# laiviet/ed-gated-gcn

Measured on AMD Instinct MI355X. Metric: gated_gcn_forward_edges_per_sec, higher is better.
Workload: dtype f32 (fp16 MFMA + block-scaled fp8 correction MFMA, fp32 accumulate)

## Files before the change

### ed-gated-gcn_amd/_capi.py

```python
import ctypes
import os

_HERE = os.path.dirname(os.path.abspath(__file__))
_LIB = None

c_i32, c_i64, c_vp, c_sz = ctypes.c_int, ctypes.c_int64, ctypes.c_void_p, ctypes.c_size_t

PROTOTYPES = {
    "ggcn_abi_version": (c_i32, []),
    "ggcn_has_f16mx6": (c_i32, []),
    "ggcn_last_error": (ctypes.c_char_p, []),
    "ggcn_csr_workspace_bytes": (c_sz, [c_i64]),
    "ggcn_csr_from_dense": (c_i32, [c_vp, c_i32, c_i32, c_i32, c_i64, c_i64, c_i64, c_vp, c_vp, c_vp,
                                    c_i64, c_vp, c_vp, c_vp, c_vp]),
    "ggcn_rowmask_from_dense": (c_i32, [c_vp, c_i32, c_i32, c_i32, c_i64, c_i64, c_i64, c_vp, c_vp, c_vp]),
    "ggcn_csr_transpose": (c_i32, [c_vp, c_vp, c_vp, c_i32, c_i32, c_vp, c_vp, c_vp, c_vp, c_vp]),
    "ggcn_csr_rowmask": (c_i32, [c_vp, c_vp, c_i32, c_i32, c_vp, c_vp]),
    "ggcn_graph_edge_lists_bytes": (c_sz, [c_i32]),
    "ggcn_graph_edge_lists": (c_i32, [c_vp, c_i32, c_i32, c_vp, c_vp]),
    "ggcn_graph_operands_bytes": (c_sz, [c_i32]),
    "ggcn_graph_operands": (c_i32, [c_vp, c_i32, c_i32, c_vp, c_vp]),
    "ggcn_graph_operands2_bytes": (c_sz, [c_i32]),
    "ggcn_graph_operands2": (c_i32, [c_vp, c_i32, c_i32, c_i32, c_vp, c_vp]),
    "ggcn_graph_operands_weighted": (c_i32, [c_vp, c_vp, c_vp, c_i32, c_i32, c_i32, c_vp, c_vp, c_vp]),
    "ggcn_layer_fused_weighted": (c_i32, [c_vp, c_i64, c_vp, c_vp, c_vp, c_vp, c_i32, c_i32, c_i32, c_i32, c_vp, c_vp, c_vp,
                                          c_vp, c_i64, c_vp, c_vp, c_vp, c_vp, c_vp, c_i32, c_vp]),
    "ggcn_graph_operands_weighted_wide_bytes": (c_sz, [c_i32, c_i32]),
    "ggcn_graph_operands_weighted_wide": (c_i32, [c_vp, c_vp, c_vp, c_i32, c_i32, c_vp, c_vp, c_vp]),
    "ggcn_layer_fused_weighted_wide": (c_i32, [c_vp, c_i64, c_vp, c_vp, c_vp, c_i32, c_i32, c_i32, c_i32, c_vp, c_vp, c_vp,
                                               c_vp, c_i64, c_vp, c_vp, c_i32, c_vp]),
    "ggcn_layer_fused_weighted_drop": (c_i32, [c_vp, c_i64, c_vp, c_vp, c_vp, c_vp, c_i32, c_i32, c_i32, c_i32, c_vp, c_vp, c_vp,
                                               c_vp, c_i64, c_vp, c_vp, c_i32, ctypes.c_float, ctypes.c_uint64, c_i32, c_i32, c_i32, c_vp]),
    "ggcn_layer_fused_weighted_wide_drop": (c_i32, [c_vp, c_i64, c_vp, c_vp, c_vp, c_i32, c_i32, c_i32, c_i32, c_vp, c_vp, c_vp,
                                                    c_vp, c_i64, c_vp, c_vp, c_i32, ctypes.c_float, ctypes.c_uint64, c_i32, c_i32, c_i32, c_vp]),
    "ggcn_layer_fused": (c_i32, [c_vp, c_i64, c_vp, c_vp, c_vp, c_vp, c_i32, c_i32, c_i32, c_i32, c_vp, c_vp, c_vp,
                                 c_vp, c_i64, c_vp, c_vp, c_vp, c_vp, c_vp, c_i32, c_vp]),
    "ggcn_layer_fused_prebias": (c_i32, [c_vp, c_i64, c_vp, c_vp, c_vp, c_vp, c_i32, c_i32, c_i32, c_i32, c_vp, c_vp, c_vp,
                                         c_vp, c_i64, c_vp, c_vp, c_i32, c_vp]),
    "ggcn_block_fused": (c_i32, [c_vp, c_i64, c_vp, c_vp, c_vp, c_vp, c_vp, c_vp, c_vp, c_i32, c_i32, c_i32, c_i32,
                                 c_vp, c_vp, c_vp, c_i64, c_vp, c_i64, c_vp, c_vp, c_vp, c_vp, c_i32, c_vp]),
    "ggcn_graph_operands2_weighted": (c_i32, [c_vp, c_vp, c_vp, c_i32, c_i32, c_i32, c_vp, c_vp, c_vp]),
    "ggcn_block_fused_weighted": (c_i32, [c_vp, c_i64, c_vp, c_vp, c_vp, c_vp, c_vp, c_vp, c_vp, c_vp, c_i32, c_i32, c_i32, c_i32,
                                          c_vp, c_vp, c_vp, c_i64, c_vp, c_i64, c_vp, c_vp, c_vp, c_vp, c_i32, c_vp]),
    "ggcn_overlap_reduce": (c_i32, [c_vp, c_i32, c_i32, c_vp, c_vp]),
    "ggcn_transpose": (c_i32, [c_vp, c_i32, c_i32, c_i64, c_vp, c_vp]),
    "ggcn_gate_mlp": (c_i32, [c_vp, c_i64, c_i32, c_i32, c_vp, c_vp, c_vp, c_vp, c_vp, c_vp, c_vp, c_vp, c_vp, c_vp, c_vp]),
    "ggcn_scores_head": (c_i32, [c_vp, c_i64, c_vp, c_i64, c_vp, c_i64, c_vp, c_i64, c_vp, c_vp, c_i64, c_i32, c_i32,
                                 c_i32, c_i32, c_vp, c_i64, c_vp, c_vp]),
    "ggcn_absmax": (c_i32, [c_vp, c_i32, c_i64, c_i64, c_i32, c_vp, c_vp]),
    "ggcn_range_flag": (c_i32, [c_vp, c_i32, c_vp]),
    "ggcn_debug_poison_lds": (c_i32, [ctypes.c_uint32, c_vp]),
    "ggcn_lab_block_fused8": (c_i32, [c_vp, c_i64, c_vp, c_vp, c_vp, c_vp, c_vp, c_vp, c_vp, c_i32, c_i32, c_i32, c_i32, c_vp, c_vp,
                                      c_vp, c_i64, c_vp, c_vp, c_vp, c_vp, c_vp, c_vp]),
    "ggcn_debug_mfma_calibrate": (c_i32, [c_i32, c_i32, c_vp, c_vp, c_vp]),
    "ggcn_debug_block_fused_stamped": (c_i32, [c_vp, c_i64, c_vp, c_vp, c_vp, c_vp, c_vp, c_vp, c_vp, c_i32, c_i32, c_i32, c_i32,
                                               c_vp, c_vp, c_vp, c_i64, c_vp, c_i64, c_vp, c_vp, c_vp, c_vp, c_i32, c_vp, c_vp]),
    "ggcn_subword_pool": (c_i32, [c_vp, c_i64, c_i64, c_i64, c_vp, c_i64, c_i64, c_vp, c_i64, c_i64,
                                  c_i32, c_i32, c_i32, c_i32, c_vp]),
    "ggcn_subword_pool_bf16": (c_i32, [c_vp, c_i64, c_i64, c_i64, c_vp, c_i64, c_i64, c_vp, c_i64, c_i64,
                                       c_i32, c_i32, c_i32, c_i32, c_vp]),
    "ggcn_linear_bf16": (c_i32, [c_vp, c_i64, c_vp, c_vp, c_i64, c_i64, c_i32, c_i32, c_vp]),
    "ggcn_linear_out_bf16": (c_i32, [c_vp, c_i64, c_vp, c_vp, c_i64, c_i64, c_i32, c_i32, c_vp]),
    "ggcn_layer_fused_bf16": (c_i32, [c_vp, c_i64, c_vp, c_vp, c_vp, c_i32, c_i32, c_i32, c_i32, c_vp, c_vp, c_vp,
                                      c_vp, c_i64, c_vp, c_vp, c_vp, c_vp, c_vp, c_vp]),
    "ggcn_layer_fused_bf16_drop": (c_i32, [c_vp, c_i64, c_vp, c_vp, c_vp, c_i32, c_i32, c_i32, c_i32, c_vp, c_vp, c_vp,
                                           c_vp, c_i64, c_vp, c_vp, c_vp, c_vp, c_vp,
                                           ctypes.c_float, ctypes.c_uint64, c_i32, c_i32, c_i32, c_vp]),
    "ggcn_layer_fused_bf16_wide": (c_i32, [c_vp, c_i64, c_vp, c_vp, c_vp, c_vp, c_i32, c_i32, c_i32, c_i32, c_vp, c_vp, c_vp,
                                           c_vp, c_i64, c_vp, c_vp, c_vp, c_vp, c_vp,
                                           ctypes.c_float, ctypes.c_uint64, c_i32, c_i32, c_i32, c_vp]),
    "ggcn_block_fused_bf16": (c_i32, [c_vp, c_i64, c_vp, c_vp, c_vp, c_vp, c_vp, c_vp, c_vp, c_i32, c_i32, c_i32, c_i32,
                                      c_vp, c_vp, c_vp, c_i64, c_vp, c_i64, c_vp, c_vp, c_vp, c_vp, c_vp]),
    "ggcn_aggregate_bf16": (c_i32, [c_vp, c_i64, c_vp, c_vp, c_vp, c_i32, c_i32, c_i32, c_vp, c_i64, c_vp]),
    "ggcn_dweight_bf16_workspace_bytes": (c_sz, [c_i64, c_i32, c_i32]),
    "ggcn_dweight_bf16": (c_i32, [c_vp, c_i64, c_vp, c_i64, c_i64, c_i32, c_i32, c_vp, c_i64, c_vp, c_vp]),
    "ggcn_weight_pack_bytes": (c_sz, [c_i32, c_i32, c_i32]),
    "ggcn_weight_pack": (c_i32, [c_vp, c_i64, c_i32, c_i32, c_i32, c_i32, c_vp, c_vp]),
    "ggcn_linear": (c_i32, [c_vp, c_i64, c_vp, c_i64, c_vp, c_vp, c_i64, c_i64, c_i32, c_i32, c_i32, c_vp]),
    "ggcn_aggregate": (c_i32, [c_vp, c_i64, c_vp, c_vp, c_vp, c_vp, c_i32, c_i32, c_i32, c_vp, c_vp, c_vp,
                               c_vp, c_i64, c_vp, c_vp, c_vp]),
    "ggcn_gate_pool_backward": (c_i32, [c_vp, c_i64, c_vp, c_vp, c_vp, c_vp, c_i64, c_vp, c_vp, c_i32, c_i32, c_i32,
                                        c_vp, c_i64, c_vp, c_vp, c_vp, c_vp, c_vp]),
    "ggcn_gate_pool_backward_drop": (c_i32, [c_vp, c_i64, c_vp, c_vp, c_vp, c_vp, c_i64, c_vp, c_vp, c_i32, c_i32, c_i32,
                                             c_vp, c_i64, c_vp, c_vp, c_vp, c_vp, ctypes.c_float, ctypes.c_uint64, c_i32, c_i32, c_i32, c_vp]),
    "ggcn_gate_pool_backward_agg": (c_i32, [c_vp, c_i64, c_vp, c_vp, c_vp, c_vp, c_i64, c_vp, c_vp, c_vp, c_i32, c_i32, c_i32,
                                            c_vp, c_i64, c_vp, c_vp, c_vp, c_vp, ctypes.c_float, ctypes.c_uint64, c_i32, c_i32, c_i32, c_vp, c_vp]),
    "ggcn_rowmask_transpose": (c_i32, [c_vp, c_i32, c_i32, c_vp, c_vp]),
    "ggcn_gate_pool_backward_mma": (c_i32, [c_vp, c_i64, c_vp, c_vp, c_vp, c_vp, c_i64, c_vp, c_vp, c_vp, c_vp, c_i32, c_i32, c_i32,
                                            c_vp, c_i64, c_vp, c_vp, c_vp, c_vp, c_vp, c_vp]),
    "ggcn_graph_operands_weighted_t_bytes": (c_sz, [c_i32]),
    "ggcn_graph_operands_weighted_t": (c_i32, [c_vp, c_vp, c_vp, c_i32, c_i32, c_vp, c_vp, c_vp]),
    "ggcn_gate_pool_backward_weighted": (c_i32, [c_vp, c_i64, c_vp, c_vp, c_vp, c_vp, c_i64, c_vp, c_vp, c_vp, c_vp, c_i32, c_i32, c_i32,
                                                 c_vp, c_i64, c_vp, c_i64, c_vp, c_vp, c_vp, c_vp, c_vp]),
    "ggcn_gate_pool_backward_weighted_drop": (c_i32, [c_vp, c_i64, c_vp, c_vp, c_vp, c_vp, c_i64, c_vp, c_vp, c_vp, c_vp, c_i32, c_i32, c_i32,
                                                      c_vp, c_i64, c_vp, c_i64, c_vp, c_vp, c_vp, c_vp,
                                                      ctypes.c_float, ctypes.c_uint64, c_i32, c_i32, c_i32, c_vp]),
    "ggcn_linear_scaled": (c_i32, [c_vp, c_i64, c_vp, c_vp, c_i64, c_i64, c_i32, c_i32, c_vp, c_vp]),
    "ggcn_layer_fused_drop": (c_i32, [c_vp, c_i64, c_vp, c_vp, c_vp, c_vp, c_i32, c_i32, c_i32, c_i32, c_vp, c_vp, c_vp,
                                      c_vp, c_i64, c_vp, c_vp, c_i32, ctypes.c_float, ctypes.c_uint64, c_i32, c_i32, c_i32, c_vp]),
    "ggcn_dropout_mask": (c_i32, [c_i64, c_i32, ctypes.c_float, ctypes.c_uint64, c_i32, c_vp, c_vp]),
    "ggcn_colsum_workspace_bytes": (c_sz, [c_i32]),
    "ggcn_colsum": (c_i32, [c_vp, c_i64, c_i64, c_i32, c_vp, c_vp, c_vp]),
    "ggcn_dweight_workspace_bytes": (c_sz, [c_i64, c_i32, c_i32, c_i32]),
    "ggcn_dweight": (c_i32, [c_vp, c_i64, c_vp, c_i64, c_i64, c_i32, c_i32, c_vp, c_i64, c_i32, c_vp, c_vp]),
    "ggcn_inv_denominators": (c_i32, [c_vp, c_vp, c_i64, c_vp, c_vp]),
    "ggcn_aggregate_t": (c_i32, [c_vp, c_i64, c_vp, c_vp, c_vp, c_vp, c_i32, c_i32, c_i32, c_vp, c_i64, c_vp]),
    "ggcn_adjacency_grad": (c_i32, [c_vp, c_i64, c_vp, c_i64, c_vp, c_vp, c_vp, c_vp, c_i32, c_i32, c_i32, c_vp, c_vp]),
    "ggcn_linear_h": (c_i32, [c_vp, c_i64, c_vp, c_vp, c_i64, c_i64, c_i32, c_i32, c_i32, c_vp]),
    "ggcn_aggregate_h": (c_i32, [c_vp, c_i64, c_vp, c_vp, c_vp, c_vp, c_i32, c_i32, c_i32, c_vp, c_vp, c_vp,
                                 c_vp, c_i64, c_vp, c_vp, c_vp]),
    "ggcn_layer_fused_h": (c_i32, [c_vp, c_i64, c_vp, c_vp, c_vp, c_vp, c_vp, c_i32, c_i32, c_i32, c_i32, c_vp, c_vp, c_vp,
                                   c_vp, c_i64, c_vp, c_vp, c_vp]),
    "ggcn_block_fused_form": (c_i32, [c_i32, c_i32, c_i32, c_i32]),
    "ggcn_dense_head": (c_i32, [c_vp, c_i64, c_vp, c_i64, c_vp, c_i32, c_i32, c_i32, c_vp, c_i64, c_vp, c_i32, c_vp, c_vp]),
    "ggcn_dense_head_signal": (c_i32, [c_vp, c_i64, c_vp, c_i64, c_vp, c_i32, c_i32, c_i32, c_vp, c_i64, c_vp, c_i32, c_vp, c_vp, c_vp]),
    "ggcn_overlap_workspace_bytes": (c_sz, [c_i32]),
    "ggcn_gate_overlap": (c_i32, [c_vp, c_vp, c_i32, c_i32, c_vp, c_vp, c_vp]),
}

ABI_VERSION = 14
PREC = {"bf16x3": 0, "fp32": 1, "f16mx8": 2, "f16": 3, "f16mx6": 4}
PACKED = ("bf16x3", "f16mx8", "f16", "f16mx6")
FLAG_WEIGHTED = 1
RANGE_OVERFLOW, RANGE_WINDOW, RANGE_HIDDEN = 1, 2, 4


def has_f16mx6():
    return bool(load_library().ggcn_has_f16mx6())


def lib_path():
    return os.environ.get("GGCN_LIB", os.path.join(_HERE, "libggcn_hip.so"))


def load_library():
    global _LIB
    if _LIB is not None:
        return _LIB
    path = lib_path()
    if not os.path.exists(path):
        raise RuntimeError(
            "libggcn_hip.so not found at %s: build it with `python -c 'import __graft_entry__ as g; "
            "g.build()'` or `make -C ed-gated-gcn_amd/csrc` (no CPU fallback exists)" % path)
    lib = ctypes.CDLL(path)
    for name, (res, args) in PROTOTYPES.items():
        fn = getattr(lib, name)
        fn.restype, fn.argtypes = res, args
    if lib.ggcn_abi_version() != ABI_VERSION:
        raise RuntimeError("libggcn_hip.so ABI %d != binding ABI %d" % (lib.ggcn_abi_version(), ABI_VERSION))
    _LIB = lib
    return lib


def check(rc, what):
    if rc != 0:
        msg = load_library().ggcn_last_error().decode("utf-8", "replace")
        raise RuntimeError("%s failed (code %d): %s" % (what, rc, msg))


def ptr(t):
    return None if t is None else ctypes.c_void_p(t.data_ptr())


def stream_of(device):
    import torch
    return ctypes.c_void_p(torch.cuda.current_stream(device).cuda_stream)
```

### ed-gated-gcn_amd/csrc/capi.hip

```cpp
#include "common.h"
#include <cstdlib>
#include "dropout_hash.h"

#include <cstring>

namespace ggcn {

char *error_buffer()
{
    static thread_local char buf[512] = "";
    return buf;
}

int fail(int code, const char *fmt, ...)
{
    va_list ap;
    va_start(ap, fmt);
    vsnprintf(error_buffer(), 512, fmt, ap);
    va_end(ap);
    return code;
}

}

// ... 99 lines not shown
                             const float *bias_pre, int B, int T, int K, int F, const float *store_gate,
                             const float *pool_gate_a, const float *pool_gate_b, float *out, int64_t ldo,
                             float *pool_a, float *pool_b, int precision, ggcn_stream_t stream)
{
    if (!bias_pre) return fail(GGCN_EINVAL, "ggcn_layer_fused_prebias: null bias_pre (ggcn_layer_fused is the plain form)");
    return layer_fused(X, ldx, wpack, rowmask, nullptr, bias, B, T, K, F, store_gate, pool_gate_a, pool_gate_b, out,
                       ldo, pool_a, pool_b, nullptr, nullptr, nullptr, precision, as_stream(stream), nullptr, bias_pre);
}

int ggcn_graph_operands_weighted(const int32_t *rowptr, const int32_t *colidx, const float *vals, int B, int T, int plane,
                                 void *graph_opsw, int32_t *flag, ggcn_stream_t stream)
{
    return graph_operands_weighted(rowptr, colidx, vals, B, T, plane, graph_opsw, flag, as_stream(stream));
}

int ggcn_layer_fused_weighted(const float *X, int64_t ldx, const void *wpack, const void *graph_opsw, const float *bias,
                              const float *zero_mid, int B, int T, int K, int F, const float *store_gate,
                              const float *pool_gate_a, const float *pool_gate_b, float *out, int64_t ldo, float *pool_a,
                              float *pool_b, float *overlap_partial, const float *overlap_in, float *overlap_out, int precision,
                              ggcn_stream_t stream)
{
    return layer_fused_weighted(X, ldx, wpack, graph_opsw, bias, zero_mid, B, T, K, F, store_gate, pool_gate_a, pool_gate_b, out, ldo,
                                pool_a, pool_b, overlap_partial, overlap_in, overlap_out, precision, as_stream(stream));
}

size_t ggcn_graph_operands_weighted_wide_bytes(int B, int T) { return graph_operands_weighted_wide_bytes(B, T); }

int ggcn_graph_operands_weighted_wide(const int32_t *rowptr, const int32_t *colidx, const float *vals, int B, int T, void *graph_opsww,
                                      int32_t *flag, ggcn_stream_t stream)
{
    return graph_operands_weighted_wide(rowptr, colidx, vals, B, T, graph_opsww, flag, as_stream(stream));
}

int ggcn_layer_fused_weighted_wide(const float *X, int64_t ldx, const void *wpack, const void *graph_opsww, const float *bias,
                                   int B, int T, int K, int F, const float *store_gate, const float *pool_gate_a,
                                   const float *pool_gate_b, float *out, int64_t ldo, float *pool_a, float *pool_b, int precision,
                                   ggcn_stream_t stream)
{
    return layer_fused_weighted_wide(X, ldx, wpack, graph_opsww, bias, B, T, K, F, store_gate, pool_gate_a, pool_gate_b, out, ldo,
                                     pool_a, pool_b, precision, as_stream(stream));
}

int ggcn_layer_fused_weighted_drop(const float *X, int64_t ldx, const void *wpack, const void *graph_opsw, const float *bias,
                                   const float *zero_mid, int B, int T, int K, int F, const float *store_gate,
                                   const float *pool_gate_a, const float *pool_gate_b, float *out, int64_t ldo, float *pool_a,
                                   float *pool_b, int precision, float p, uint64_t seed, int sel_store, int sel_a, int sel_b,
                                   ggcn_stream_t stream)
{
    if (int rc = drop_entry_checks("ggcn_layer_fused_weighted_drop", p, sel_store, sel_a, sel_b)) return rc;
    const DropSpec d = make_drop_spec(p, seed, sel_store, sel_a, sel_b);
    return layer_fused_weighted_drop(X, ldx, wpack, graph_opsw, bias, zero_mid, B, T, K, F, store_gate, pool_gate_a, pool_gate_b, out, ldo,
                                     pool_a, pool_b, precision, as_stream(stream), &d);
}

int ggcn_layer_fused_weighted_wide_drop(const float *X, int64_t ldx, const void *wpack, const void *graph_opsww, const float *bias,
                                        int B, int T, int K, int F, const float *store_gate, const float *pool_gate_a,
                                        const float *pool_gate_b, float *out, int64_t ldo, float *pool_a, float *pool_b, int precision,
                                        float p, uint64_t seed, int sel_store, int sel_a, int sel_b, ggcn_stream_t stream)
{
    if (int rc = drop_entry_checks("ggcn_layer_fused_weighted_wide_drop", p, sel_store, sel_a, sel_b)) return rc;
    const DropSpec d = make_drop_spec(p, seed, sel_store, sel_a, sel_b);
    return layer_fused_weighted_wide(X, ldx, wpack, graph_opsww, bias, B, T, K, F, store_gate, pool_gate_a, pool_gate_b, out, ldo,
                                     pool_a, pool_b, precision, as_stream(stream), &d);
}

int ggcn_gate_pool_backward_weighted_drop(const float *out, int64_t ldo, const float *store_gate, const float *gate_a,
                                          const float *gate_b, const float *d_out, int64_t ldd, const float *d_pa, const float *d_pb,
                                          const void *graph_ops_wt, const float *inv, int B, int T, int F, float *dH, int64_t ldh,
                                          float *dY, int64_t ldy, float *d_sg, float *d_ga, float *d_gb, float *d_bsum, float p,
                                          uint64_t seed, int sel_store, int sel_a, int sel_b, ggcn_stream_t stream)
{
    if (int rc = drop_entry_checks("ggcn_gate_pool_backward_weighted_drop", p, sel_store, sel_a, sel_b)) return rc;
    const DropSpec d = make_drop_spec(p, seed, sel_store, sel_a, sel_b);
    return gate_pool_backward_weighted(out, ldo, store_gate, gate_a, gate_b, d_out, ldd, d_pa, d_pb, graph_ops_wt, inv, B, T, F, dH, ldh,
                                       dY, ldy, d_sg, d_ga, d_gb, d_bsum, as_stream(stream), &d);
}

int ggcn_block_fused(const float *X, int64_t ldx, const void *wpack1, const void *wpack12, const void *graph_ops,
                     const void *graph_ops2, const float *bias1, const float *bias_mid, const float *bias2, int B, int T, int K, int F,
                     const float *gate1, const float *gate2, float *gcn1, int64_t ld1, float *x_out, int64_t ld2,
                     float *x1, float *y1, float *pool_out, float *overlap_partial, int precision,
                     ggcn_stream_t stream)
{
    return block_fused(X, ldx, wpack1, wpack12, graph_ops, graph_ops2, bias1, bias_mid, bias2, B, T, K, F, gate1, gate2, gcn1, ld1,
                       x_out, ld2, x1, y1, pool_out, overlap_partial, precision, as_stream(stream));
}

int ggcn_graph_operands2_weighted(const int32_t *rowptr, const int32_t *colidx, const float *vals, int B, int T, int plane,
                                  void *graph_ops2w, int32_t *flag, ggcn_stream_t stream)
{
    return graph_operands2_weighted(rowptr, colidx, vals, B, T, plane, graph_ops2w, flag, as_stream(stream));
}

int ggcn_block_fused_weighted(const float *X, int64_t ldx, const void *wpack1, const void *wpack12, const void *graph_opsw,
                              const void *graph_ops2w, const float *bias1, const float *bias_mid, const float *bias2,
                              const float *zero_mid, int B, int T, int K, int F, const float *gate1, const float *gate2, float *gcn1,
                              int64_t ld1, float *x_out, int64_t ld2, float *x1, float *y1, float *pool_out, float *overlap_partial,
                              int precision, ggcn_stream_t stream)
{
    return block_fused_weighted(X, ldx, wpack1, wpack12, graph_opsw, graph_ops2w, bias1, bias_mid, bias2, zero_mid, B, T, K, F, gate1,
                                gate2, gcn1, ld1, x_out, ld2, x1, y1, pool_out, overlap_partial, precision, as_stream(stream));
}

int ggcn_overlap_reduce(const float *partials, int B, int F, float *xy, ggcn_stream_t stream)
{
    return overlap_reduce(partials, B, F, xy, as_stream(stream));
}

size_t ggcn_weight_pack_bytes(int K, int F, int precision) { return weight_pack_bytes(K, F, precision); }

int ggcn_weight_pack(const float *W, int64_t ldw, int K, int F, int precision, int transposed, void *wpack,
                     ggcn_stream_t stream)
{
    return weight_pack(W, ldw, K, F, precision, transposed != 0, wpack, as_stream(stream));
}

int ggcn_aggregate_t(const float *G, int64_t ldg, const int32_t *rowptr_t, const int32_t *colidx_t,
                     const float *vals_t, const float *src_scale, int B, int T, int F, float *out, int64_t ldo,
                     ggcn_stream_t stream)
{
    return aggregate_t(G, ldg, rowptr_t, colidx_t, vals_t, src_scale, B, T, F, out, ldo, as_stream(stream));
}

int ggcn_inv_denominators(const int32_t *rowptr, const float *vals, int64_t n_rows, float *inv,
                          ggcn_stream_t stream)
{
    return inv_denominators(rowptr, vals, n_rows, inv, as_stream(stream));
}

int ggcn_adjacency_grad(const float *dY, int64_t ldy, const float *hidden, int64_t ldh, const float *inv, const int32_t *rowptr,
                        const int32_t *colidx, const float *vals, int B, int T, int F, float *d_adj, ggcn_stream_t stream)
{
    return adjacency_grad(dY, ldy, hidden, ldh, inv, rowptr, colidx, vals, B, T, F, d_adj, as_stream(stream));
}

int ggcn_linear(const float *X, int64_t ldx, const float *W, int64_t ldw, const void *wpack, float *Y,
                int64_t ldy, int64_t M, int K, int F, int precision, ggcn_stream_t stream)
{
    if (int rc = linear_entry_checks("ggcn_linear", !X || !Y, M, K, F, ldx, ldy)) return rc;
    switch (precision) {
        case GGCN_PREC_BF16X3:
        case GGCN_PREC_F16MX8:
            return linear_packed(X, ldx, wpack, Y, ldy, M, K, F, precision, as_stream(stream));
        case GGCN_PREC_FP32:
            if (!W) return fail(GGCN_EINVAL, "ggcn_linear(fp32): W is NULL");
            if (ldw < F) return fail(GGCN_EINVAL, "ggcn_linear(fp32): ldw < F");
            return linear_fp32(X, ldx, W, ldw, Y, ldy, M, K, F, as_stream(stream));
        default:
            return fail(GGCN_EINVAL, "ggcn_linear: unknown precision %d", precision);
    }
}

int ggcn_linear_bf16(const void *X, int64_t ldx, const void *wpack, float *Y, int64_t ldy, int64_t M, int K, int F,
                     ggcn_stream_t stream)
{
    if (int rc = linear_entry_checks("ggcn_linear_bf16", !X || !Y || !wpack, M, K, F, ldx, ldy)) return rc;
    if (reinterpret_cast<uintptr_t>(X) % 2 || reinterpret_cast<uintptr_t>(Y) % 4)
        return fail(GGCN_EINVAL, "ggcn_linear_bf16: X / Y not aligned to their element size");
    return linear_bf16(X, ldx, wpack, Y, ldy, M, K, F, as_stream(stream));
}

int ggcn_linear_out_bf16(const float *X, int64_t ldx, const void *wpack, void *Y, int64_t ldy, int64_t M, int K, int F,
                         ggcn_stream_t stream)
{
    if (int rc = linear_entry_checks("ggcn_linear_out_bf16", !X || !Y || !wpack, M, K, F, ldx, ldy)) return rc;
    if (reinterpret_cast<uintptr_t>(X) % 4 || reinterpret_cast<uintptr_t>(Y) % 2)
        return fail(GGCN_EINVAL, "ggcn_linear_out_bf16: X / Y not aligned to their element size");
    return linear_out_bf16(X, ldx, wpack, Y, ldy, M, K, F, as_stream(stream));
}
// ... 179 lines not shown

int ggcn_layer_fused_drop(const float *X, int64_t ldx, const void *wpack, const uint32_t *rowmask, const void *graph_ops,
                          const float *bias, int B, int T, int K, int F, const float *store_gate,
                          const float *pool_gate_a, const float *pool_gate_b, float *out, int64_t ldo,
                          float *pool_a, float *pool_b, int precision, float p, uint64_t seed, int sel_store,
                          int sel_a, int sel_b, ggcn_stream_t stream)
{
    if (int rc = drop_entry_checks("ggcn_layer_fused_drop", p, sel_store, sel_a, sel_b)) return rc;
    const DropSpec d = make_drop_spec(p, seed, sel_store, sel_a, sel_b);
    return layer_fused(X, ldx, wpack, rowmask, graph_ops, bias, B, T, K, F, store_gate, pool_gate_a, pool_gate_b, out,
                       ldo, pool_a, pool_b, nullptr, nullptr, nullptr, precision, as_stream(stream), &d);
}

int ggcn_dropout_mask(int64_t rows, int F, float p, uint64_t seed, int stream_id, float *mask, ggcn_stream_t stream)
{
    return dropout_mask(rows, F, p, seed, stream_id, mask, as_stream(stream));
}

size_t ggcn_colsum_workspace_bytes(int F) { return colsum_workspace_bytes(F); }

int ggcn_colsum(const float *X, int64_t ld, int64_t M, int F, float *out, void *workspace, ggcn_stream_t stream)
{
    return colsum(X, ld, M, F, out, workspace, as_stream(stream));
}

size_t ggcn_dweight_workspace_bytes(int64_t n_rows, int K, int F, int precision)
{
    return precision == GGCN_PREC_FP32 ? dweight_workspace_bytes(n_rows, K, F) : dweight_bx3_workspace_bytes(n_rows, K, F);
}

int ggcn_dweight(const float *X, int64_t ldx, const float *dH, int64_t ldg, int64_t n_rows, int K, int F,
                 float *dW, int64_t lddw, int precision, void *workspace, ggcn_stream_t stream)
{
    if (precision == GGCN_PREC_FP32)
        return dweight(X, ldx, dH, ldg, n_rows, K, F, dW, lddw, workspace, as_stream(stream));
    if (precision != GGCN_PREC_BF16X3)
        return fail(GGCN_EUNSUPPORTED, "ggcn_dweight: precision %d (gradients need fp32 range: use bf16x3 or fp32)", precision);
    return dweight_bx3(X, ldx, dH, ldg, n_rows, K, F, dW, lddw, workspace, as_stream(stream));
}

size_t ggcn_dweight_bf16_workspace_bytes(int64_t n_rows, int K, int F) { return dweight_bf16_workspace_bytes(n_rows, K, F); }

int ggcn_dweight_bf16(const void *X, int64_t ldx, const float *dH, int64_t ldg, int64_t n_rows, int K, int F, float *dW,
                      int64_t lddw, void *workspace, ggcn_stream_t stream)
{
    if (X && reinterpret_cast<uintptr_t>(X) % 2) return fail(GGCN_EINVAL, "ggcn_dweight_bf16: X not 2-byte aligned");
    return dweight_bf16(X, ldx, dH, ldg, n_rows, K, F, dW, lddw, workspace, as_stream(stream));
}

int ggcn_subword_pool_bf16(const float *A, int64_t sa_b, int64_t sa_r, int64_t sa_c, const void *X, int64_t x_batch,
                           int64_t ldx, void *Y, int64_t y_batch, int64_t ldy, int B, int R, int C, int D,
                           ggcn_stream_t stream)
{
    return subword_pool_bf16(A, sa_b, sa_r, sa_c, X, x_batch, ldx, Y, y_batch, ldy, B, R, C, D, as_stream(stream));
}

int ggcn_subword_pool(const float *A, int64_t sa_b, int64_t sa_r, int64_t sa_c, const float *X, int64_t x_batch,
                      int64_t ldx, float *Y, int64_t y_batch, int64_t ldy, int B, int R, int C, int D,
                      ggcn_stream_t stream)
{
    return subword_pool(A, sa_b, sa_r, sa_c, X, x_batch, ldx, Y, y_batch, ldy, B, R, C, D, as_stream(stream));
}

int ggcn_absmax(const void *X, int is_half, int64_t ld, int64_t M, int K, float *out, ggcn_stream_t stream)
{
    return absmax(X, is_half, ld, M, K, out, as_stream(stream));
}

int ggcn_debug_poison_lds(uint32_t pattern, ggcn_stream_t stream) { return poison_lds(pattern, as_stream(stream)); }

int ggcn_debug_mfma_calibrate(int n_wg, int stages, uint64_t *stamps, float *sink, ggcn_stream_t stream)
{
    return mfma_calibrate(n_wg, stages, reinterpret_cast<unsigned long long *>(stamps), sink, as_stream(stream));
}

int ggcn_debug_block_fused_stamped(const float *X, int64_t ldx, const void *wpack1, const void *wpack12, const void *graph_ops,
                                   const void *graph_ops2, const float *bias1, const float *bias_mid, const float *bias2, int B,
                                   int T, int K, int F, const float *gate1, const float *gate2, float *gcn1, int64_t ld1,
                                   float *x_out, int64_t ld2, float *x1, float *y1, float *pool_out, float *overlap_partial,
                                   int precision, uint64_t *stamps, ggcn_stream_t stream)
{
    if (!stamps) return fail(GGCN_EINVAL, "ggcn_debug_block_fused_stamped: null stamp buffer");
    return block_fused(X, ldx, wpack1, wpack12, graph_ops, graph_ops2, bias1, bias_mid, bias2, B, T, K, F, gate1, gate2, gcn1, ld1,
                       x_out, ld2, x1, y1, pool_out, overlap_partial, precision, as_stream(stream),
                       reinterpret_cast<unsigned long long *>(stamps));
}

int ggcn_range_flag(uint32_t *flag, int clear, ggcn_stream_t stream)
{
    if (!flag) return fail(GGCN_EINVAL, "ggcn_range_flag: null flag pointer");
    int rc = range_flag_linear(flag, clear, as_stream(stream));
    rc = rc ? rc : range_flag_fused(flag, clear, as_stream(stream));
    rc = rc ? rc : range_flag_wide(flag, clear, as_stream(stream));
    rc = rc ? rc : range_flag_wide8(flag, clear, as_stream(stream));
    rc = rc ? rc : range_flag_block8(flag, clear, as_stream(stream));
    rc = rc ? rc : range_flag_weighted_drop(flag, clear, as_stream(stream));
#ifdef GGCN_WITH_F16MX6
    rc = rc ? rc : range_flag_fused6(flag, clear, as_stream(stream));
#endif
    return rc;
}

int ggcn_transpose(const float *W, int rows, int cols, int64_t ldw, float *Wt, ggcn_stream_t stream)
{
    return transpose_f32(W, rows, cols, ldw, Wt, as_stream(stream));
}

int ggcn_gate_mlp(const float *aspect, int64_t lda, int B, int H, const float *w1t_a, const float *b1_a,
                  const float *w2t_a, const float *b2_a, float *gate_a, const float *w1t_b, const float *b1_b,
                  const float *w2t_b, const float *b2_b, float *gate_b, ggcn_stream_t stream)
{
    return gate_mlp(aspect, lda, B, H, w1t_a, b1_a, w2t_a, b2_a, gate_a, w1t_b, b1_b, w2t_b, b2_b, gate_b, as_stream(stream));
}

int ggcn_scores_head(const float *X, int64_t ldx, const float *aspect, int64_t lda, const float *logits, int64_t ldl,
                     const float *fc_weight, int64_t ldw, const float *fc_bias, const float *dist, int64_t ldd, int B,
                     int T, int H, int C, float *scores, int64_t ld_scores, float *kl_part, ggcn_stream_t stream)
{
    return scores_head(X, ldx, aspect, lda, logits, ldl, fc_weight, ldw, fc_bias, dist, ldd, B, T, H, C, scores, ld_scores,
                       kl_part, as_stream(stream));
}

int ggcn_dense_head(const float *pooled, int64_t ldp, const float *Wt, int64_t ldw, const float *bias, int B, int H, int C,
                    float *logits, int64_t ldl, const float *overlap_partials, int F_block, float *xy, ggcn_stream_t stream)
{
    return dense_head(pooled, ldp, Wt, ldw, bias, B, H, C, logits, ldl, overlap_partials, F_block, xy, as_stream(stream));
}

int ggcn_dense_head_signal(const float *pooled, int64_t ldp, const float *Wt, int64_t ldw, const float *bias, int B, int H, int C,
                           float *logits, int64_t ldl, const float *overlap_partials, int F_block, float *xy, uint32_t *signal,
                           ggcn_stream_t stream)
{
    if (!signal) return fail(GGCN_EINVAL, "ggcn_dense_head_signal: null signal words (ggcn_dense_head is the plain form)");
    return dense_head(pooled, ldp, Wt, ldw, bias, B, H, C, logits, ldl, overlap_partials, F_block, xy, as_stream(stream), signal);
}

size_t ggcn_overlap_workspace_bytes(int B) { return overlap_workspace_bytes(B); }

int ggcn_gate_overlap(const float *x1, const float *y1, int B, int F, float *xy, void *workspace,
                      ggcn_stream_t stream)
{
    return gate_overlap(x1, y1, B, F, xy, workspace, as_stream(stream));
}

}
```

### ed-gated-gcn_amd/csrc/common.h

```cpp
#pragma once
#include <hip/hip_runtime.h>
#include <cstdarg>
#include <cstdint>
#include <cstdio>

#include "../../include/ggcn.h"

namespace ggcn {

struct DropSpec;
constexpr int kWave = 64;

char *error_buffer();
int fail(int code, const char *fmt, ...);

inline hipStream_t as_stream(ggcn_stream_t s) { return reinterpret_cast<hipStream_t>(s); }

inline int check_launch(const char *what) {
    hipError_t e = hipGetLastError();
    if (e != hipSuccess) return fail(GGCN_ELAUNCH, "%s: %s", what, hipGetErrorString(e));
    return GGCN_OK;
}

inline bool aligned16(const void *p) { return (reinterpret_cast<uintptr_t>(p) & 15u) == 0; }
// ... 10 lines not shown
int linear_fp32(const float *X, int64_t ldx, const float *W, int64_t ldw, float *Y, int64_t ldy,
                int64_t M, int K, int F, hipStream_t st);

size_t weight_pack_bytes(int K, int F, int precision);
int weight_pack(const float *W, int64_t ldw, int K, int F, int precision, bool transposed, void *wpack, hipStream_t st);
int linear_packed(const float *X, int64_t ldx, const void *wpack, float *Y, int64_t ldy,
                  int64_t M, int K, int F, int precision, hipStream_t st);

bool linear_scaled_takes(const float *X, int64_t ldx, const float *Y, int64_t ldy, int K, int F);
int linear_scaled(const float *X, int64_t ldx, const void *wpack, float *Y, int64_t ldy, int64_t M, int K, int F, const float *amax,
                  hipStream_t st);
int linear_packed_h(const void *X, int64_t ldx, const void *wpack, void *Y, int64_t ldy, int64_t M, int K,
                    int F, int precision, hipStream_t st);
int linear_bf16(const void *X, int64_t ldx, const void *wpack, float *Y, int64_t ldy, int64_t M, int K, int F, hipStream_t st);
int linear_out_bf16(const float *X, int64_t ldx, const void *wpack, void *Y, int64_t ldy, int64_t M, int K, int F, hipStream_t st);
int aggregate_t(const float *G, int64_t ldg, const int32_t *rowptr_t, const int32_t *colidx_t,
                const float *vals_t, const float *src_scale, int B, int T, int F, float *out, int64_t ldo,
                hipStream_t st);
int inv_denominators(const int32_t *rowptr, const float *vals, int64_t n, float *inv, hipStream_t st);
int adjacency_grad(const float *dY, int64_t ldy, const float *hidden, int64_t ldh, const float *inv, const int32_t *rowptr,
                   const int32_t *colidx, const float *vals, int B, int T, int F, float *d_adj, hipStream_t st);
int aggregate_h(const void *Hd, int64_t ldh, const int32_t *rowptr, const int32_t *colidx, const float *vals,
                const float *bias, int B, int T, int F, const float *store_gate, const float *pool_gate_a,
                const float *pool_gate_b, void *out, int64_t ldo, float *pool_a, float *pool_b, hipStream_t st);

int layer_fused_h(const void *X, int64_t ldx, const void *wpack, const int32_t *rowptr, const int32_t *colidx,
                  const float *vals, const float *bias, int B, int T, int K, int F, const float *store_gate,
                  const float *pool_gate_a, const float *pool_gate_b, void *out, int64_t ldo, float *pool_a,
                  float *pool_b, hipStream_t st);

int aggregate(const float *Hd, int64_t ldh, const int32_t *rowptr, const int32_t *colidx,
              const float *vals, const float *bias, int B, int T, int F, const float *store_gate,
              const float *pool_gate_a, const float *pool_gate_b, float *out, int64_t ldo,
              float *pool_a, float *pool_b, hipStream_t st);

int aggregate_bf16(const void *X, int64_t ldx, const int32_t *rowptr, const int32_t *colidx, const float *vals, int B, int T, int K,
                   float *Z, int64_t ldz, hipStream_t st);

int subword_pool(const float *A, int64_t sa_b, int64_t sa_r, int64_t sa_c, const float *X, int64_t x_batch,
                 int64_t ldx, float *Y, int64_t y_batch, int64_t ldy, int B, int R, int C, int D, hipStream_t st);
int subword_pool_bf16(const float *A, int64_t sa_b, int64_t sa_r, int64_t sa_c, const void *X, int64_t x_batch,
                      int64_t ldx, void *Y, int64_t y_batch, int64_t ldy, int B, int R, int C, int D, hipStream_t st);
int csr_rowmask(const int32_t *rowptr, const int32_t *colidx, int B, int T, uint32_t *rowmask, hipStream_t st);
int graph_operands(const uint32_t *rowmask, int B, int T, void *ops, hipStream_t st);
int graph_edge_lists(const uint32_t *rowmask, int B, int T, void *lists, hipStream_t st);
int graph_operands2(const uint32_t *rowmask, int B, int T, int plane, void *ops2, hipStream_t st);
int graph_operands_weighted(const int32_t *rowptr, const int32_t *colidx, const float *vals, int B, int T, int plane, void *ops,
                            int *flag, hipStream_t st);
int layer_fused_weighted(const float *X, int64_t ldx, const void *wpack, const void *graph_opsw, const float *bias, const float *zero_mid,
                         int B, int T, int K, int F, const float *store_gate, const float *pool_gate_a, const float *pool_gate_b,
                         float *out, int64_t ldo, float *pool_a, float *pool_b, float *overlap_partial, const float *overlap_in,
                         float *overlap_out, int precision, hipStream_t st);
size_t graph_operands_weighted_wide_bytes(int B, int T);
int graph_operands_weighted_wide(const int32_t *rowptr, const int32_t *colidx, const float *vals, int B, int T, void *ops, int *flag,
                                 hipStream_t st);
int layer_fused_weighted_wide(const float *X, int64_t ldx, const void *wpack, const void *ops, const float *bias, int B, int T, int K, int F,
                              const float *store_gate, const float *pool_gate_a, const float *pool_gate_b, float *out, int64_t ldo,
                              float *pool_a, float *pool_b, int precision, hipStream_t st, const struct DropSpec *drop = nullptr);
int layer_fused_weighted_drop(const float *X, int64_t ldx, const void *wpack, const void *graph_opsw, const float *bias, const float *zero_mid,
                              int B, int T, int K, int F, const float *store_gate, const float *pool_gate_a, const float *pool_gate_b,
                              float *out, int64_t ldo, float *pool_a, float *pool_b, int precision, hipStream_t st, const struct DropSpec *drop);
int layer_fused(const float *X, int64_t ldx, const void *wpack, const uint32_t *rowmask, const void *graph_ops, const float *bias,
                int B, int T, int K, int F, const float *store_gate, const float *pool_gate_a,
                const float *pool_gate_b, float *out, int64_t ldo, float *pool_a, float *pool_b,
                float *overlap_partial, const float *overlap_in, float *overlap_out, int precision, hipStream_t st,
                const struct DropSpec *drop = nullptr, const float *bias_pre = nullptr);
int layer_fused_bf16(const char *who, const void *X, int64_t ldx, const void *wpack, const uint32_t *rowmask, const void *graph_ops,
                     const float *bias, int B, int T, int K, int F,
                     const float *store_gate, const float *pool_gate_a, const float *pool_gate_b, float *out, int64_t ldo,
                     float *pool_a, float *pool_b, float *overlap_partial, const float *overlap_in, float *overlap_out,
                     hipStream_t st, const struct DropSpec *drop = nullptr);
int block_fused_bf16(const void *X, int64_t ldx, const void *wpack1, const void *wpack12, const void *graph_ops, const void *graph_ops2,
                     const float *bias1, const float *bias_mid, const float *bias2, int B, int T, int K, int F,
                     const float *gate1, const float *gate2, float *gcn1, int64_t ld1, float *x_out, int64_t ld2,
                     float *x1, float *y1, float *pool_out, float *overlap_partial, hipStream_t st);
int graph_operands2_weighted(const int32_t *rowptr, const int32_t *colidx, const float *vals, int B, int T, int plane, void *ops2,
                             int *flag, hipStream_t st);
int block_fused_weighted(const float *X, int64_t ldx, const void *wpack1, const void *wpack12, const void *graph_opsw,
                         const void *graph_ops2w, const float *bias1, const float *bias_mid, const float *bias2, const float *zero_mid,
                         int B, int T, int K, int F, const float *gate1, const float *gate2, float *gcn1, int64_t ld1, float *x_out,
                         int64_t ld2, float *x1, float *y1, float *pool_out, float *overlap_partial, int precision, hipStream_t st);
int dropout_mask(int64_t rows, int F, float p, uint64_t seed, int sel, float *out, hipStream_t st);

int block_fused(const float *X, int64_t ldx, const void *wpack1, const void *wpack12, const void *graph_ops, const void *graph_ops2,
                const float *bias1, const float *bias_mid, const float *bias2, int B, int T, int K, int F,
                const float *gate1, const float *gate2, float *gcn1, int64_t ld1, float *x_out, int64_t ld2,
                float *x1, float *y1, float *pool_out, float *overlap_partial, int precision, hipStream_t st,
                unsigned long long *stamps = nullptr);
int mfma_calibrate(int n_wg, int stages, unsigned long long *stamps, float *sink, hipStream_t st);
int overlap_reduce(const float *partials, int B, int F, float *xy, hipStream_t st);

int gate_pool_backward(const float *out, int64_t ldo, const float *store_gate, const float *gate_a,
                       const float *gate_b, const float *d_out, int64_t ldd, const float *d_pa,
                       const float *d_pb, int B, int T, int F, float *dY, int64_t ldy, float *d_sg,
                       float *d_ga, float *d_gb, float *d_bsum, hipStream_t st, const struct DropSpec *drop = nullptr);
int gate_pool_backward_agg(const float *out, int64_t ldo, const float *store_gate, const float *gate_a,
                           const float *gate_b, const float *d_out, int64_t ldd, const float *d_pa,
                           const float *d_pb, const uint32_t *rowmask, int B, int T, int F, float *dH, int64_t ldh,
                           float *d_sg, float *d_ga, float *d_gb, float *d_bsum, hipStream_t st, const struct DropSpec *drop = nullptr,
                           float *dh_amax = nullptr);
int rowmask_transpose(const uint32_t *rowmask, int B, int T, uint32_t *rowmask_t, hipStream_t st);
int gate_pool_backward_mma(const float *out, int64_t ldo, const float *store_gate, const float *gate_a, const float *gate_b,
                           const float *d_out, int64_t ldd, const float *d_pa, const float *d_pb, const void *graph_ops,
                           const void *graph_ops_t, int B, int T, int F, float *dH, int64_t ldh, float *d_sg, float *d_ga,
                           float *d_gb, float *d_bsum, float *dh_amax, hipStream_t st);
size_t graph_operands_weighted_t_bytes(int B);
int graph_operands_weighted_t(const int32_t *rowptr, const int32_t *colidx, const float *vals, int B, int T, void *ops, int *flag,
                              hipStream_t st);
int gate_pool_backward_weighted(const float *out, int64_t ldo, const float *store_gate, const float *gate_a, const float *gate_b,
                                const float *d_out, int64_t ldd, const float *d_pa, const float *d_pb, const void *graph_ops_wt,
                                const float *inv, int B, int T, int F, float *dH, int64_t ldh, float *dY, int64_t ldy, float *d_sg,
                                float *d_ga, float *d_gb, float *d_bsum, hipStream_t st, const struct DropSpec *drop = nullptr);
size_t colsum_workspace_bytes(int F);
int colsum(const float *X, int64_t ld, int64_t M, int F, float *out, void *workspace, hipStream_t st);

size_t dweight_workspace_bytes(int64_t N, int K, int F);
size_t dweight_bx3_workspace_bytes(int64_t N, int K, int F);
bool dweight_tn_takes(const float *X, int64_t ldx, const float *G, int64_t ldg, int64_t N, int K, int F);
size_t dweight_tn_workspace_bytes(int64_t N, int K, int F);
int dweight_tn(const float *X, int64_t ldx, const float *G, int64_t ldg, int64_t N, int K, int F, float *dW, int64_t lddw,
               void *workspace, hipStream_t st);
int dweight_bx3(const float *X, int64_t ldx, const float *G, int64_t ldg, int64_t N, int K, int F, float *dW,
                int64_t lddw, void *workspace, hipStream_t st);
size_t dweight_bf16_workspace_bytes(int64_t N, int K, int F);
int dweight_bf16(const void *X, int64_t ldx, const float *G, int64_t ldg, int64_t N, int K, int F, float *dW,
                 int64_t lddw, void *workspace, hipStream_t st);
int weight_pack_rows(const float *W, int64_t ldw, int64_t K_valid, int F, int k_steps_total, void *pack, hipStream_t st);
int dweight(const float *X, int64_t ldx, const float *G, int64_t ldg, int64_t N, int K, int F, float *dW,
            int64_t lddw, void *workspace, hipStream_t st);

int absmax(const void *X, int is_half, int64_t ld, int64_t M, int K, float *out, hipStream_t st);
int poison_lds(uint32_t pattern, hipStream_t st);
int range_flag_linear(unsigned int *dst, int clear, hipStream_t st);
int range_flag_fused(unsigned int *dst, int clear, hipStream_t st);
int range_flag_wide(unsigned int *dst, int clear, hipStream_t st);
int range_flag_wide8(unsigned int *dst, int clear, hipStream_t st);
int range_flag_block8(unsigned int *dst, int clear, hipStream_t st);
int range_flag_weighted_drop(unsigned int *dst, int clear, hipStream_t st);
int lab_block_fused8(const float *X, int64_t ldx, const void *wpack1, const void *wpack12, const void *graph_ops, const void *graph_ops2,
                     const float *bias1, const float *bias_mid, const float *bias2, int B, int T, int K, int F, const float *gate1,
                     const float *gate2, float *x_out, int64_t ld2, float *x1, float *y1, float *pool_out, float *overlap_partial,
                     hipStream_t st, unsigned long long *stamps = nullptr, int flags = 0);
constexpr int kBlock8RowMajor = 1, kBlock8NoDma = 2, kBlock8SameSlots = 4, kBlock8Product = 8;
bool block8_shape(int B, int T, int K, int F);
bool block8_takes(const float *X, int64_t ldx, const void *wpack1, const void *wpack12, int B, int T, int K, int F, const float *gate1,
                  const float *gate2, const float *bias1, const float *bias_mid, const float *bias2, const void *graph_ops,
                  const void *graph_ops2, const float *x_out, int64_t ld2);
int range_flag_fused6(unsigned int *dst, int clear, hipStream_t st);

int transpose_f32(const float *W, int rows, int cols, int64_t ldw, float *Wt, hipStream_t st);
int gate_mlp(const float *aspect, int64_t lda, int B, int H, const float *w1t_a, const float *b1_a, const float *w2t_a,
             const float *b2_a, float *gate_a, const float *w1t_b, const float *b1_b, const float *w2t_b,
             const float *b2_b, float *gate_b, hipStream_t st);
int scores_head(const float *X, int64_t ldx, const float *aspect, int64_t lda, const float *logits, int64_t ldl,
                const float *fcw, int64_t ldw, const float *fcb, const float *dist, int64_t ldd, int B, int T, int H,
                int C, float *scores, int64_t lds_, float *kl_part, hipStream_t st);

int dense_head(const float *pooled, int64_t ldp, const float *Wt, int64_t ldw, const float *bias, int B, int H, int C,
               float *logits, int64_t ldl, const float *partials, int F_block, float *xy, hipStream_t st, unsigned *signal = nullptr);

size_t overlap_workspace_bytes(int B);
int gate_overlap(const float *x1, const float *y1, int B, int F, float *xy, void *workspace,
                 hipStream_t st);

}
```

### ed-gated-gcn_amd/csrc/fused_block8.hip

```cpp
#include "fused_common.h"

#include <cstdlib>

namespace ggcn {
namespace {

constexpr int kB8Threads = 512;
constexpr int kB8Lds = kLdsBytes + 2 * kEpiLdsBytes;

__device__ __forceinline__ bool getenv_slot_same(const FusedArgs &a) { return (a.k_steps & 0x20000000) != 0; }

template <int BASE>
__device__ __forceinline__ float staged_mid_max(const char *lds, bool dma, int lane)
{
    if (dma) {
        const float4 m4 = *reinterpret_cast<const float4 *>(lds + EpiLds<BASE>::kBias + BN * 4 + lane * 16);
        float mm = fmaxf(fmaxf(fabsf(m4.x), fabsf(m4.y)), fmaxf(fabsf(m4.z), fabsf(m4.w)));
#pragma unroll
        for (int d = 32; d >= 1; d >>= 1) mm = fmaxf(mm, __shfl_xor(mm, d));
        return mm;
    }
    const float4 mm = *reinterpret_cast<const float4 *>(lds + EpiLds<BASE>::kMidMax);
    return fmaxf(fmaxf(mm.x, mm.y), fmaxf(mm.z, mm.w));
}

template <bool FULLT, bool VST>
__global__ __launch_bounds__(kB8Threads, 1) void block_fused8_kernel(const FusedArgs a)
{
    extern __shared__ __attribute__((aligned(16))) char lds[];
    const int B = a.B, T = a.T, K = a.K, F = a.F;
    int n_wgi, g_tile;
    if (a.n_parts == 2) {
        const int xcd = blockIdx.x & 7, qb = blockIdx.x >> 3;
        const int total = a.g_tiles * a.n_wg, per_xcd = (total + 7) >> 3;
        const int w = xcd * per_xcd + qb;
        if (qb >= per_xcd || w >= total) return;
        n_wgi = w / a.g_tiles;
        g_tile = w - n_wgi * a.g_tiles;
    } else {
        if (!tile_of_block(blockIdx.x, a.g_tiles, a.n_wg, g_tile, n_wgi)) return;
    }

    const int tid8 = threadIdx.x;
    const unsigned long long t_start = a.stamps ? __builtin_amdgcn_s_memrealtime() : 0;
    const int group = __builtin_amdgcn_readfirstlane(tid8 >> 8);
    const int tid = tid8 & 255;
    const int wave = __builtin_amdgcn_readfirstlane(tid >> 6);
    const LayerPart &lp = a.part[group];
    const int gt0 = g_tile * 4, g0 = gt0;
    const int n_tiles_total = (F + NT - 1) / NT;
    const int nt0 = n_wgi * (BN / NT) + wave * RN;

    constexpr int NP = Geom<float>::NP;
    const float *arow[NP];
    bool avalid[NP];
    int rel[NP];
#pragma unroll
    for (int i = 0; i < NP; ++i) {
        const int row = stage_row<float>(i < 2 ? i + 2 * group : 0);
        const int g = gt0 + (row >> 5), r = row & 31;
        avalid[i] = i < 2 && (g < B) && (FULLT || r < T);
        arow[i] = a.X;
        rel[i] = avalid[i] ? (row >> 5) * T + (row & 31) : -1;
    }
    const bool dma = (a.n_wg * BN == F) && (gt0 + 4 <= B) && a.ov_in == nullptr && a.ov_out == nullptr && (a.k_steps & 0x40000000) != 0;
    const int k_steps = a.k_steps & 0x1fffffff;
    if (dma) {
        if (group == 0) stage_epilogue_operands_dma<kLdsBytes>(a, lp, g0, n_wgi, lds, tid);
        else stage_epilogue_operands_dma<kLdsBytes + kEpiLdsBytes>(a, lp, g0, n_wgi, lds, tid);
    } else {
        if (group == 0) stage_epilogue_operands<kLdsBytes>(a, lp, g0, n_wgi, lds, tid);
        else stage_epilogue_operands<kLdsBytes + kEpiLdsBytes>(a, lp, g0, n_wgi, lds, tid);
    }

    f32x16 acc[4][RN];
    float amax;
    const int64_t pack_bytes = (int64_t)n_tiles_total * (k_steps / 2) * mx8::STAGE_PACK_BYTES;
    const float bw1 = *reinterpret_cast<const float *>(a.part[0].wpack + pack_bytes);
    const float bw12 = *reinterpret_cast<const float *>(a.part[1].wpack + pack_bytes);
    const unsigned long long t_loop0 = a.stamps ? __builtin_amdgcn_s_memrealtime() : 0;
    mx8::BufX<float> bx = mx8::make_bufx<float>(a.X, a.ldx, (int64_t)gt0 * T, (int64_t)B * T, rel, tid);
    if (group == 0 || getenv_slot_same(a))
        mx8::mainloop<float, true, true, !FULLT, false, true, 4, false, 2, 0>(arow, avalid, lp.wpack, K, k_steps / 2, 0, nt0, n_tiles_total, lds, acc, 0, 4,
                                                                               &amax, &bx, 1.0f, 2 * group);
    else
        mx8::mainloop<float, true, true, !FULLT, false, true, 4, false, 2, 2>(arow, avalid, lp.wpack, K, k_steps / 2, 0, nt0, n_tiles_total, lds, acc, 0, 4,
                                                                               &amax, &bx, 1.0f, 2 * group);
    unsigned long long t_loop1 = 0;
    if (a.stamps) { asm volatile("" :: "v"(acc[3][RN - 1][15])); t_loop1 = __builtin_amdgcn_s_memrealtime(); }
    mx8::range_verdict(amax, bw12, staged_mid_max<kLdsBytes + kEpiLdsBytes>(lds, dma, tid & 63), true);
    mx8::range_verdict(amax, bw1, 0.0f, false);
    if (group == 0) {
        epilogue<1, FULLT, VST, false, false, kLdsBytes>(a, lp, acc, g0, nt0, n_tiles_total, lds, tid);
    } else {
        if (lp.out) epilogue<1, FULLT, VST, true, true, kLdsBytes + kEpiLdsBytes>(a, lp, acc, g0, nt0, n_tiles_total, lds, tid);
        else epilogue<1, FULLT, VST, true, false, kLdsBytes + kEpiLdsBytes>(a, lp, acc, g0, nt0, n_tiles_total, lds, tid);
    }
    if (a.stamps && tid == 0) {
        unsigned long long *o = a.stamps + ((size_t)blockIdx.x * 2 + group) * 4;
        o[0] = t_start; o[1] = t_loop0; o[2] = t_loop1; o[3] = __builtin_amdgcn_s_memrealtime();
    }
}

}

int device_cu_count()
{
    static int cus = 0;
    if (cus == 0) {
        int dev = 0, n = 0;
        if (hipGetDevice(&dev) != hipSuccess || hipDeviceGetAttribute(&n, hipDeviceAttributeMultiprocessorCount, dev) != hipSuccess || n <= 0) n = 256;
        cus = n;
    }
    return cus;
}
bool block8_shape(int B, int T, int K, int F)
{
    if (B <= 0 || T > 32 || T <= 0 || F <= 0 || K <= 0 || F % BN != 0 || K % BK != 0) return false;
    const int64_t total = (int64_t)((B + 3) / 4) * (F / BN), cus = device_cu_count();
    return total >= 6 * cus || (total >= 3 * cus && total % cus == 0);
}
bool block8_takes(const float *X, int64_t ldx, const void *wpack1, const void *wpack12, int B, int T, int K, int F, const float *gate1,
                  const float *gate2, const float *bias1, const float *bias_mid, const float *bias2, const void *graph_ops,
                  const void *graph_ops2, const float *x_out, int64_t ld2)
{
    if (!block8_shape(B, T, K, F)) return false;
    if (ldx < K || !aligned16(wpack1) || !aligned16(wpack12) || (x_out && ld2 < F)) return false;
    if (!((ldx % 4 == 0) && aligned16(X) && (int64_t)ldx * 4 * 257 < ((int64_t)1 << 31))) return false;
    if (!graph_ops || !graph_ops2 || !gate1 || !gate2 || !bias_mid) return false;
    if (!(aligned16(gate1) && aligned16(gate2) && aligned16(bias1) && aligned16(bias2) && aligned16(bias_mid) && aligned16(graph_ops) &&
          aligned16(graph_ops2)))
        return false;
    if (x_out && !((ld2 % 4 == 0) && aligned16(x_out) && (int64_t)T * ld2 * 4 < ((int64_t)1 << 31))) return false;
    return true;
}

int lab_block_fused8(const float *X, int64_t ldx, const void *wpack1, const void *wpack12, const void *graph_ops, const void *graph_ops2,
                     const float *bias1, const float *bias_mid, const float *bias2, int B, int T, int K, int F, const float *gate1,
                     const float *gate2, float *x_out, int64_t ld2, float *x1, float *y1, float *pool_out, float *overlap_partial,
                     hipStream_t st, unsigned long long *stamps, int flags)
{
    const char *who = (flags & kBlock8Product) ? "ggcn_block_fused" : "ggcn_lab_block_fused8";
    if (!X || !wpack1 || !wpack12 || !graph_ops || !graph_ops2 || !gate1 || !gate2 || !x1 || !y1 || !bias_mid)
        return fail(GGCN_EINVAL, "%s: null pointer", who);
    if (B <= 0 || T <= 0 || T > 32 || K <= 0 || F <= 0) return fail(GGCN_EUNSUPPORTED, "%s: B=%d T=%d K=%d F=%d (graphs of <= 32 nodes)", who, B, T, K, F);
    if (ldx < K) return fail(GGCN_EINVAL, "%s: ldx < K", who);
    if (!aligned16(wpack1) || !aligned16(wpack12)) return fail(GGCN_EINVAL, "%s: wpack must be 16-byte aligned", who);
    if (x_out && ld2 < F) return fail(GGCN_EINVAL, "%s: leading dimension of the output too small", who);
    const bool avec = (K % 4 == 0) && (ldx % 4 == 0) && aligned16(X) && (int64_t)ldx * 4 * 257 < ((int64_t)1 << 31);
    if (!avec || K % BK != 0) return fail(GGCN_EUNSUPPORTED, "%s: fast shapes only (K %% 32 == 0, 16-byte aligned rows)", who);
    if (!x_out && !pool_out) return fail(GGCN_EINVAL, "%s: neither x nor its pool requested", who);
    FusedArgs a = {};
    a.X = X; a.ldx = ldx; a.graph_ops = static_cast<const char *>(graph_ops); a.graph_ops2 = static_cast<const char *>(graph_ops2);
    const bool rowmajor = (flags & kBlock8RowMajor) != 0;
    a.B = B; a.T = T; a.K = K; a.F = F; a.n_parts = rowmajor ? 3 : 2;
    a.part[0] = LayerPart{static_cast<const char *>(wpack1), bias1, nullptr, nullptr, nullptr, gate1, gate2, nullptr, x1, y1, overlap_partial, 0};
    a.part[1] = LayerPart{static_cast<const char *>(wpack12), bias2, bias_mid, nullptr, gate2, gate2, nullptr, x_out, pool_out, nullptr, nullptr, (int)ld2};
    a.stamps = stamps;
    a.k_steps = round_up(K, BK) / KSTEP;
    const bool al = (F % 4 == 0) && aligned16(gate1) && aligned16(gate2) && aligned16(bias1) && aligned16(bias2) && aligned16(bias_mid) &&
                    aligned16(graph_ops) && aligned16(graph_ops2) && !(flags & kBlock8NoDma);
    if (al) a.k_steps |= 0x40000000;
    if (flags & kBlock8SameSlots) a.k_steps |= 0x20000000;
    a.n_wg = (F + BN - 1) / BN;
    a.g_tiles = (B + 3) / 4;
    const bool vst = x_out && (F % 4 == 0) && (ld2 % 4 == 0) && aligned16(x_out) && (int64_t)T * ld2 * 4 < ((int64_t)1 << 31);
    if (x_out && !vst) return fail(GGCN_EUNSUPPORTED, "%s: x needs F %% 4 == 0 and 16-byte aligned rows", who);
    const bool fullt = (T == 32) && (B % 4 == 0);
    const int64_t total = (int64_t)a.g_tiles * a.n_wg;
    const int64_t grid = rowmajor ? grid_for(a.g_tiles, a.n_wg) : 8 * ((total + 7) / 8);
    if (grid > (int64_t)INT32_MAX) return fail(GGCN_EUNSUPPORTED, "%s: batch too large", who);
#define GGCN_L8(FT, VS)                                                                                                           \
    do {                                                                                                                          \
        auto kern = block_fused8_kernel<FT, VS>;                                                                                  \
        if (hipFuncSetAttribute(reinterpret_cast<const void *>(kern), hipFuncAttributeMaxDynamicSharedMemorySize, kB8Lds) != hipSuccess) \
            return fail(GGCN_ELAUNCH, "%s: cannot reserve %d bytes of LDS", who, kB8Lds);                                         \
        hipLaunchKernelGGL(kern, dim3((unsigned)grid), dim3(kB8Threads), kB8Lds, st, a);                                          \
    } while (0)
    if (fullt && vst) GGCN_L8(true, true);
    else if (fullt) GGCN_L8(true, false);
    else if (vst) GGCN_L8(false, true);
    else GGCN_L8(false, false);
#undef GGCN_L8
    return check_launch(who);
}

GGCN_RANGE_FLAG_TU(range_flag_block8)

}
```

### ed-gated-gcn_amd/csrc/fused_common.h

```cpp
#pragma once
#include "f16mx8_core.h"
#include "dropout_hash.h"
#include "lab_hooks.h"

namespace ggcn {

struct LayerPart {
    const char *wpack;
    const float *bias;
    const float *mid;
    const float *pre;
    const float *store_gate;
    const float *pool_gate_a;
    const float *pool_gate_b;
    float *out;
    float *pool_a, *pool_b;
    float *ov_partial;
    int ldo;
};

struct FusedArgs {
    const float *X;
    int64_t ldx;
    const uint32_t *rowmask;
    const char *graph_ops;
    const char *graph_ops2;
    const float *ov_in;
    float *ov_out;
    int B, T, K, F;
    int g_tiles, n_wg, n_parts, k_steps;
    LayerPart part[2];
    DropSpec drop;
    unsigned long long *stamps;
    const __bf16 *Xb;
};


int launch_fused_wide(const char *who, const FusedArgs &a, int precision, int sb, bool fast, bool vst, int64_t grid, hipStream_t st);
int launch_fused_wide8(const char *who, const FusedArgs &a, int precision, bool fast, bool vst, int64_t grid, hipStream_t st);
int launch_fused6(const char *who, const FusedArgs &a, bool fullt, bool vst, int64_t grid, hipStream_t st);
int launch_fused_weighted_drop(const char *who, const FusedArgs &a, int precision, bool avec, bool kfull, bool fullt, bool vst, int64_t grid,
                               hipStream_t st);
int launch_fused_block_weighted(const char *who, const FusedArgs &a, int precision, bool avec, bool kfull, bool fullt, bool vst, int64_t grid,
                                hipStream_t st);

namespace {

using namespace bx3;

template <typename XT>
__device__ __forceinline__ const XT *fused_x(const FusedArgs &a)
{
    if constexpr (std::is_same<XT, float>::value) return a.X;
    else return a.Xb;
}

__device__ __forceinline__ void split2(const f32x16 &acc, bf16x8 (&frag)[2][2])
{
#pragma unroll
    for (int s = 0; s < 2; ++s)
#pragma unroll
        for (int j = 0; j < 8; ++j) {
            const float v = acc[8 * s + j];
            const __bf16 p0 = (__bf16)v;
            frag[0][s][j] = p0;
            frag[1][s][j] = (__bf16)(v - (float)p0);
        }
}

__device__ __forceinline__ void store_out4(float *p, const float4 &v)
{
#if GGCN_LAB_NT_STORE
    typedef float f4 __attribute__((ext_vector_type(4)));
    __builtin_nontemporal_store(f4{v.x, v.y, v.z, v.w}, reinterpret_cast<f4 *>(p));
#else
    *reinterpret_cast<float4 *>(p) = v;
#endif
}

__device__ __forceinline__ void store_out4_stream(float *p, const float4 &v)
{
    typedef float f4 __attribute__((ext_vector_type(4)));
    __builtin_nontemporal_store(f4{v.x, v.y, v.z, v.w}, reinterpret_cast<f4 *>(p));
}

__device__ __forceinline__ float upper_half_to_lower(float v)
{
    const auto r = __builtin_amdgcn_permlane32_swap(__float_as_uint(v), __float_as_uint(v), false, false);
    return __uint_as_float(r[1]);
}

__device__ __forceinline__ void expand_mask(uint32_t mh, bf16x8 (&af)[2])
{
    typedef unsigned short u16x2 __attribute__((ext_vector_type(2)));
    typedef short i16x2 __attribute__((ext_vector_type(2)));
    union { bf16x8 v; uint32_t w[4]; } u[2];
#pragma unroll
    for (int s = 0; s < 2; ++s) {
        const uint32_t m16 = s == 0 ? (mh & 0xFFFFu) : (mh >> 16);
        const u16x2 both = __builtin_bit_cast(u16x2, m16 | (m16 << 16));
#pragma unroll
        for (int q = 0; q < 4; ++q) {
            const int b = 8 * (q >> 1) + 2 * (q & 1);
            const u16x2 top = both << u16x2{(unsigned short)(15 - b), (unsigned short)(14 - b)};
            const i16x2 spread = __builtin_bit_cast(i16x2, top) >> i16x2{15, 15};
            u[s].w[q] = __builtin_bit_cast(uint32_t, spread) & 0x3F803F80u;
        }
    }
    af[0] = u[0].v;
    af[1] = u[1].v;
}

__device__ __forceinline__ f32x16 adj_times(const bf16x8 (&af)[2], const f32x16 &t)
{
    bf16x8 hfrag[2][2];
    split2(t, hfrag);
    f32x16 y;
// ... 137 lines not shown
__device__ __forceinline__ void fused_range_verdict(float amax, const char *wpack, int64_t pack_bytes, const char *lds, bool window)
{
    const float bw = *reinterpret_cast<const float *>(wpack + pack_bytes);
    const float4 mm = *reinterpret_cast<const float4 *>(lds + EpiLds<BASE>::kMidMax);
    mx8::range_verdict(amax, bw, fmaxf(fmaxf(mm.x, mm.y), fmaxf(mm.z, mm.w)), window);
}

template <int BASE, bool GIVEN = false>
__device__ __forceinline__ void stage_epilogue_operands_dma(const FusedArgs &a, const LayerPart &lp, int g0, int n_wgi, char *lds, int tid,
                                                            const char *given = nullptr)
{
    constexpr int kEpiOps = EpiLds<BASE>::kOps, kEpiGate = EpiLds<BASE>::kGate, kEpiBias = EpiLds<BASE>::kBias;
    const int lane = tid & 63, wave = __builtin_amdgcn_readfirstlane(tid >> 6);
    const int F = a.F;
    const bool second = GIVEN || lp.mid != nullptr;
    const int total = 4 * (second ? kOps2Bytes : kOpsBytes);
    const char *src = (GIVEN ? given : second ? a.graph_ops2 : a.graph_ops) + (int64_t)g0 * (second ? kOps2Bytes : kOpsBytes);
    for (int piece = wave; piece * 1024 < total; piece += 4)
        if (piece * 1024 + lane * 16 < total)
            __builtin_amdgcn_global_load_lds((const __attribute__((address_space(1))) void *)(src + piece * 1024 + lane * 16),
                                             (__attribute__((address_space(3))) void *)(lds + kEpiOps + piece * 1024), 16, 0, 0);
    const float *gp[3] = {lp.store_gate, lp.pool_gate_a, lp.pool_gate_b};
    float *gl = reinterpret_cast<float *>(lds + kEpiGate);
#pragma unroll
    for (int k = 0; k < 3; ++k) {
        if (gp[k]) {
            __builtin_amdgcn_global_load_lds((const __attribute__((address_space(1))) void *)(gp[k] + (int64_t)(g0 + wave) * F + n_wgi * BN + lane * 4),
                                             (__attribute__((address_space(3))) void *)(lds + kEpiGate + ((k * 4 + wave) * BN) * 4), 16, 0, 0);
        } else {
#pragma unroll
            for (int i = 0; i < 4; ++i) gl[(k * 4 + i) * BN + tid] = 1.0f;
        }
    }
    float *bl = reinterpret_cast<float *>(lds + kEpiBias);
    if (lp.bias) {
        if (wave == 0) __builtin_amdgcn_global_load_lds((const __attribute__((address_space(1))) void *)(lp.bias + n_wgi * BN + lane * 4),
                                                        (__attribute__((address_space(3))) void *)(lds + kEpiBias), 16, 0, 0);
    } else bl[tid] = 0.0f;
    if (lp.mid) {
        if (wave == 1) __builtin_amdgcn_global_load_lds((const __attribute__((address_space(1))) void *)(lp.mid + n_wgi * BN + lane * 4),
                                                        (__attribute__((address_space(3))) void *)(lds + kEpiBias + BN * 4), 16, 0, 0);
    } else bl[BN + tid] = 0.0f;
}
template <int BASE>
__device__ __forceinline__ void dma_range_verdict(float amax, const char *wpack, int64_t pack_bytes, const char *lds, int lane)
{
    const float4 m4 = *reinterpret_cast<const float4 *>(lds + EpiLds<BASE>::kBias + BN * 4 + lane * 16);
    float mm = fmaxf(fmaxf(fabsf(m4.x), fabsf(m4.y)), fmaxf(fabsf(m4.z), fabsf(m4.w)));
#pragma unroll
    for (int d = 32; d >= 1; d >>= 1) mm = fmaxf(mm, __shfl_xor(mm, d));
    const float bw = *reinterpret_cast<const float *>(wpack + pack_bytes);
    mx8::range_verdict(amax, bw, mm, true);
}

__device__ __forceinline__ float vmax_raw(float x, float y) { float d; asm("v_max_f32 %0, %1, %2" : "=v"(d) : "v"(x), "v"(y)); return d; }
__device__ __forceinline__ float vmin_raw(float x, float y) { float d; asm("v_min_f32 %0, %1, %2" : "=v"(d) : "v"(x), "v"(y)); return d; }

__device__ __forceinline__ void meet_halves(float &vmax, float &vmin)
{
    const auto r = __builtin_amdgcn_permlane32_swap(__float_as_uint(vmax), __float_as_uint(vmin), false, false);
    const float a = __uint_as_float(r[0]), b = __uint_as_float(r[1]);
    const float m = vmax_raw(a, b), n = vmin_raw(a, b);
    const auto q = __builtin_amdgcn_permlane32_swap(__float_as_uint(n), __float_as_uint(a), false, false);
    vmax = m;
    vmin = __uint_as_float(q[1]);
}

__device__ __forceinline__ float wave_sum_to_lane0(float v)
{
    v += __uint_as_float(__builtin_amdgcn_update_dpp(0, __float_as_uint(v), 0xB1, 0xF, 0xF, true));
    v += __uint_as_float(__builtin_amdgcn_update_dpp(0, __float_as_uint(v), 0x4E, 0xF, 0xF, true));
    v += __uint_as_float(__builtin_amdgcn_update_dpp(0, __float_as_uint(v), 0x141, 0xF, 0xF, true));
    v += __uint_as_float(__builtin_amdgcn_update_dpp(0, __float_as_uint(v), 0x140, 0xF, 0xF, true));
    const float r1 = __uint_as_float(__builtin_amdgcn_readlane(__float_as_uint(v), 16));
    const float r2 = __uint_as_float(__builtin_amdgcn_readlane(__float_as_uint(v), 32));
    const float r3 = __uint_as_float(__builtin_amdgcn_readlane(__float_as_uint(v), 48));
    return (v + r1) + (r2 + r3);
}

__device__ __forceinline__ __amdgpu_buffer_rsrc_t out_rsrc(void *p)
{
    return __builtin_amdgcn_make_buffer_rsrc(p, 0, 0x7fffffff, 0x00020000);
}

template <int SCH, bool FULLT, bool VST, bool MID, bool OUT, int BASE = kLdsBytes, bool DROP = false>
__device__ __forceinline__ void epilogue(const FusedArgs &a, const LayerPart &lp, f32x16 (&acc)[4][RN], int g0, int nt0,
                                         int n_tiles_total, char *lds, int tid)
{
    constexpr int kEpiOps = EpiLds<BASE>::kOps, kEpiGate = EpiLds<BASE>::kGate, kEpiBias = EpiLds<BASE>::kBias;
    using P = AggPlane<SCH>;
    typedef typename P::frag frag;
    const int B = a.B, T = a.T, F = a.F;
    float *__restrict__ out = lp.out, *__restrict__ pool_a = lp.pool_a, *__restrict__ pool_b = lp.pool_b;
    float *__restrict__ ov_partial = lp.ov_partial;
    const int ldo = lp.ldo;
    const int lane = tid & 63;
    const int wave = __builtin_amdgcn_readfirstlane(tid >> 6);
    const int c = lane & 31, h = lane >> 5;

    const char *ops_lds = lds + kEpiOps;
    const float *gate_lds = reinterpret_cast<const float *>(lds + kEpiGate);
    const float *bias_lds = reinterpret_cast<const float *>(lds + kEpiBias);
    const int wn = wave % WN;
    float vb[RN], vmid[RN];
    bool col_ok[RN];
#pragma unroll
    for (int j = 0; j < RN; ++j) {
        col_ok[j] = (nt0 + j) * NT + c < F;
        vb[j] = bias_lds[wn * (RN * NT) + j * NT + c];
        vmid[j] = bias_lds[BN + wn * (RN * NT) + j * NT + c];
    }
    const int lane_off = 4 * h * ldo + c;
    float *stage_lds = reinterpret_cast<float *>(lds) + wave * (32 * 64);
    constexpr bool vst = VST && OUT;
    constexpr bool direct_store = !VST && OUT;

#pragma unroll
    for (int i = 0; i < 4; ++i) {
        const int g = g0 + i;
        if (!FULLT && g >= B) break;
        constexpr int kBlk = MID ? kOps2Bytes : kOpsBytes;
        constexpr int kRowOff = MID ? 4096 : 2048;
        frag afv[2], afl[2];
#pragma unroll
        for (int s = 0; s < 2; ++s) {
            const uint4 raw = *reinterpret_cast<const uint4 *>(ops_lds + i * kBlk + s * 1024 + lane * 16);
            union { frag v; uint32_t w[4]; } u;
            if constexpr (MID) {
                u.w[0] = raw.x; u.w[1] = raw.y; u.w[2] = raw.z; u.w[3] = raw.w;
                afv[s] = u.v;
                const uint4 rl = *reinterpret_cast<const uint4 *>(ops_lds + i * kBlk + 2048 + s * 1024 + lane * 16);
                u.w[0] = rl.x; u.w[1] = rl.y; u.w[2] = rl.z; u.w[3] = rl.w;
                afl[s] = u.v;
            } else {
                u.w[0] = raw.x & P::kOne; u.w[1] = raw.y & P::kOne;
                u.w[2] = raw.z & P::kOne; u.w[3] = raw.w & P::kOne;
                afv[s] = u.v;
            }
        }
        float4 rv[4];
#pragma unroll
        for (int q = 0; q < 4; ++q) rv[q] = *reinterpret_cast<const float4 *>(ops_lds + i * kBlk + kRowOff + h * 64 + q * 16);
        float vsg[RN], vga[RN], vgb[RN];
#pragma unroll
        for (int j = 0; j < RN; ++j) {
            const int at = i * BN + wn * (RN * NT) + j * NT + c;
            vsg[j] = gate_lds[at];
            vga[j] = gate_lds[4 * BN + at];
            vgb[j] = gate_lds[8 * BN + at];
        }
        bool tile_ok[RN];
#pragma unroll
        for (int j = 0; j < RN; ++j) tile_ok[j] = nt0 + j < n_tiles_total;

        f32x16 y[RN];
#pragma unroll
        for (int j = 0; j < RN; ++j) {
            frag hf[2][2];
            P::split(acc[i][j], hf);
#pragma unroll
            for (int r = 0; r < 16; ++r) y[j][r] = 0.0f;
            if constexpr (MID) {
#pragma unroll
                for (int s = 0; s < 2; ++s) y[j] = P::mma(afl[s], hf[0][s], y[j]);
#pragma unroll
                for (int s = 0; s < 2; ++s) y[j] = P::mma(afv[s], hf[1][s], y[j]);
#pragma unroll
                for (int s = 0; s < 2; ++s) y[j] = P::mma(afv[s], hf[0][s], y[j]);
            } else {
#pragma unroll
                for (int p = 1; p >= 0; --p)
#pragma unroll
                    for (int s = 0; s < 2; ++s) { if constexpr (!((GGCN_LAB_EPI) & 2)) y[j] = P::mma(afv[s], hf[p][s], y[j]); else y[j][s] += (float)hf[p][s][0]; }
            }
        }
        float rinv[16];
#pragma unroll
        for (int q = 0; q < 4; ++q) {
            rinv[4 * q] = rv[q].x; rinv[4 * q + 1] = rv[q].y; rinv[4 * q + 2] = rv[q].z; rinv[4 * q + 3] = rv[q].w;
        }
        float dot = 0.0f;
#pragma unroll
        for (int j = 0; j < RN; ++j) {
            if (!tile_ok[j]) break;
            const int gn = (nt0 + j) * NT + c;
            float vmax = -INFINITY, vmin = INFINITY, pmax_a = -INFINITY, pmax_b = -INFINITY;
            float *tile = OUT ? out + ((int64_t)g * T) * ldo + (nt0 + j) * NT : nullptr;
            const float sg = vsg[j];
            const float bj = vb[j];
            const uint32_t didx0 = DROP ? (uint32_t)(((int64_t)g * T + 4 * h) * F + gn) : 0u;
#pragma unroll
            for (int r = 0; r < 16; ++r) {
                const int row0 = (r & 3) + 8 * (r >> 2);
                const float v = MID ? fmaf(y[j][r], kM2InvScale, fmaf(rinv[r], vmid[j], bj)) : y[j][r] * rinv[r] + bj;
                float vs = v * sg;
                if constexpr (DROP) {
                    const uint32_t hh = drop_hash(didx0 + (uint32_t)(row0 * F), a.drop.seed_lo, a.drop.seed_hi);
                    vs *= drop_keep(hh, a.drop.sel[0], a.drop.thr, a.drop.scale);
                    if (FULLT || row0 + 4 * h < T) {
                        pmax_a = fmaxf(pmax_a, v * vga[j] * drop_keep(hh, a.drop.sel[1], a.drop.thr, a.drop.scale));
                        pmax_b = fmaxf(pmax_b, v * vgb[j] * drop_keep(hh, a.drop.sel[2], a.drop.thr, a.drop.scale));
                    }
                }
                if constexpr (vst) {
                    stage_lds[(row0 + 4 * h) * 64 + ((32 * j + c) ^ (32 * h))] = vs;
                }
                if (FULLT || row0 + 4 * h < T) {
                    if (direct_store && col_ok[j]) tile[lane_off + row0 * ldo] = vs;
                    if constexpr (!DROP) {
                        vmax = fmaxf(vmax, v);
                        vmin = fminf(vmin, v);
                    }
                }
            }
            float pa, pb;
            if constexpr (DROP) {
                pa = fmaxf(pmax_a, upper_half_to_lower(pmax_a));
                pb = fmaxf(pmax_b, upper_half_to_lower(pmax_b));
            } else {
                meet_halves(vmax, vmin);
                const float ga = vga[j], gb = vgb[j];
                pa = ga * (ga >= 0.0f ? vmax : vmin);
                pb = gb * (gb >= 0.0f ? vmax : vmin);
            }
            if (h == 0 && col_ok[j]) {
                if (pool_a) __builtin_amdgcn_raw_buffer_store_b32(__float_as_uint(pa), out_rsrc(pool_a + (int64_t)g * F), 4 * gn, 0, 0);
                if (pool_b) __builtin_amdgcn_raw_buffer_store_b32(__float_as_uint(pb), out_rsrc(pool_b + (int64_t)g * F), 4 * gn, 0, 0);
                dot = fmaf(pa, pb, dot);
            }
        }
        if (ov_partial && nt0 < n_tiles_total) {
            const float tot = wave_sum_to_lane0(dot);
            if (lane == 0) ov_partial[(int64_t)g * ((F + 63) / 64) + (nt0 >> 1)] = tot;
        }
        if constexpr (vst) {
            __builtin_amdgcn_fence(__ATOMIC_RELEASE, "wavefront");
            __builtin_amdgcn_wave_barrier();
            const int colq = (lane & 15) * 4;
            const int gcol = nt0 * NT + colq;
            const __amdgpu_buffer_rsrc_t orsrc = out_rsrc(out + ((int64_t)g * T) * ldo);
            const int voff = ((lane >> 4) * ldo + gcol) * 4;
#pragma unroll
            for (int it = 0; it < 8; ++it) {
                const int row = 4 * it + (lane >> 4);
                const float4 v4 = *reinterpret_cast<const float4 *>(&stage_lds[row * 64 + (colq ^ (32 * ((row >> 2) & 1)))]);
                typedef uint32_t u32x4 __attribute__((ext_vector_type(4)));
                if ((FULLT || row < T) && gcol < F && !((GGCN_LAB_EPI) & 1))
                    __builtin_amdgcn_raw_buffer_store_b128(__builtin_bit_cast(u32x4, v4), orsrc, voff, 4 * it * ldo * 4, (GGCN_LAB_NT_STORE) ? 2 : 0);
            }
            __builtin_amdgcn_fence(__ATOMIC_ACQUIRE, "wavefront");
            __builtin_amdgcn_wave_barrier();
        }
        if (i == 0) GGCN_TRACE(7);
    }
}


}
}
```

### ed-gated-gcn_amd/csrc/fused_layer.hip

```cpp
#include "fused_common.h"

#include <cstdlib>

namespace ggcn {
namespace {

__global__ __launch_bounds__(256) void graph_operands_kernel(const uint32_t *__restrict__ rowmask, int B, int T,
                                                             char *__restrict__ ops)
{
    const int lane = threadIdx.x & 63;
    const int g = blockIdx.x * 4 + (threadIdx.x >> 6);
    if (g >= B) return;
    const int r = lane & 31, h = lane >> 5;
    const uint32_t m = r < T ? rowmask[(int64_t)g * T + r] : 0u;
    char *blk = ops + (int64_t)g * kOpsBytes;
#pragma unroll
    for (int s = 0; s < 2; ++s) {
        uint32_t w[4];
#pragma unroll
        for (int q = 0; q < 4; ++q) {
            const int b = 16 * s + 8 * (q >> 1) + 2 * (q & 1) + 4 * h;
            const uint32_t two = (m >> b) & 3u;
            w[q] = (two & 1u) * 0xFFFFu + (two >> 1) * 0xFFFF0000u;
        }
        *reinterpret_cast<uint4 *>(blk + s * 1024 + lane * 16) = make_uint4(w[0], w[1], w[2], w[3]);
    }
    const int rr = lane & 15, hh = (lane >> 4) & 1;
    const int row = (rr & 3) + 8 * (rr >> 2) + 4 * hh;
    const uint32_t mrow = __shfl(m, row);
    if (lane < 32) reinterpret_cast<float *>(blk + 2048)[lane] = 1.0f / (float)(__popc(mrow) + 1);
}

template <int PLANE>
__global__ __launch_bounds__(256) void graph_operands2_kernel(const uint32_t *__restrict__ rowmask, int B, int T,
                                                              char *__restrict__ ops2)
{
    const int lane = threadIdx.x & 63;
    const int g = blockIdx.x * 4 + (threadIdx.x >> 6);
    if (g >= B) return;
    const int r = lane & 31, h = lane >> 5;
    const uint32_t m = r < T ? rowmask[(int64_t)g * T + r] : 0u;
    const float inv_r = 1.0f / (float)(__popc(m) + 1);
    float a2[2][8];
#pragma unroll
    for (int s = 0; s < 2; ++s)
#pragma unroll
        for (int e = 0; e < 8; ++e) a2[s][e] = 0.0f;
    for (int j = 0; j < T; ++j) {
        const uint32_t mj = (uint32_t)__builtin_amdgcn_readlane((int)m, j);
        const float invj = 1.0f / (float)(__popc(mj) + 1);
        if ((m >> j) & 1u) {
#pragma unroll
            for (int s = 0; s < 2; ++s)
#pragma unroll
                for (int e = 0; e < 8; ++e) {
                    const int c = 16 * s + 8 * (e >> 2) + 4 * h + (e & 3);
                    a2[s][e] += ((mj >> c) & 1u) ? invj : 0.0f;
                }
        }
    }
    char *blk = ops2 + (int64_t)g * kOps2Bytes;
#pragma unroll
    for (int s = 0; s < 2; ++s) {
        union { uint4 q; unsigned short u[8]; } hi, lo;
#pragma unroll
        for (int e = 0; e < 8; ++e) {
            const float v = a2[s][e] * inv_r * kM2Scale;
            if constexpr (PLANE == 1) {
                const _Float16 vh = (_Float16)v, vl = (_Float16)(v - (float)vh);
                hi.u[e] = __builtin_bit_cast(unsigned short, vh);
                lo.u[e] = __builtin_bit_cast(unsigned short, vl);
            } else {
                const __bf16 vh = (__bf16)v, vl = (__bf16)(v - (float)vh);
                hi.u[e] = __builtin_bit_cast(unsigned short, vh);
                lo.u[e] = __builtin_bit_cast(unsigned short, vl);
            }
        }
        *reinterpret_cast<uint4 *>(blk + s * 1024 + lane * 16) = hi.q;
        *reinterpret_cast<uint4 *>(blk + 2048 + s * 1024 + lane * 16) = lo.q;
    }
    const int rr = lane & 15, hh = (lane >> 4) & 1;
    const int row = (rr & 3) + 8 * (rr >> 2) + 4 * hh;
    const uint32_t mrow = __shfl(m, row);
    if (lane < 32) reinterpret_cast<float *>(blk + 4096)[lane] = (float)__popc(mrow) / (float)(__popc(mrow) + 1);
}
// ... 80 lines not shown
    const int n_tiles_total = (F + NT - 1) / NT;
    const int nt0 = n_wgi * (BN / NT) + wn * RN;

    constexpr int NP = Geom<XT>::NP;
    const XT *arow[NP];
    bool avalid[NP];
#pragma unroll
    for (int i = 0; i < NP; ++i) {
        const int row = stage_row<XT>(i);
        const int g = gt0 + (row >> 5), r = row & 31;
        avalid[i] = (g < B) && (FULLT || r < T);
        const int64_t node = avalid[i] ? (int64_t)g * T + r : 0;
        arow[i] = fused_x<XT>(a) + node * a.ldx;
    }

#if !GGCN_LAB_NO_DMA_STAGE
    const bool dma_stage = SCH == 1 && (a.n_wg * BN == F) && (gt0 + 4 <= B) && a.drop.thr == 0 && (F % 4 == 0) &&
                           ((reinterpret_cast<uintptr_t>(lp.store_gate) | reinterpret_cast<uintptr_t>(lp.pool_gate_a) | reinterpret_cast<uintptr_t>(lp.pool_gate_b) |
                             reinterpret_cast<uintptr_t>(lp.bias) | reinterpret_cast<uintptr_t>(lp.mid)) & 15u) == 0;
    if (dma_stage) stage_epilogue_operands_dma<kLdsBytes>(a, lp, g0, n_wgi, lds, tid);
    else
#else
    constexpr bool dma_stage = false;
#endif
    stage_epilogue_operands<kLdsBytes>(a, lp, g0, n_wgi, lds, tid);
    f32x16 acc[4][RN];
    GGCN_TRACE(4);
    unsigned long long stamp_c = 0, stamp_w = 0;
    if constexpr (STAMP) {
        stamp_c = __builtin_readcyclecounter();
        stamp_w = __builtin_amdgcn_s_memrealtime();
    }
    if constexpr (SCH == 0)
        bx3::mainloop<XT, AVEC, KFULL, !FULLT>(arow, avalid, wpack, K, a.k_steps, wm, nt0, n_tiles_total, lds, acc);
    else {
        float amax;
        constexpr bool BUF = AVEC && KFULL;
        mx8::BufX<float> bx;
        if constexpr (BUF) {
            int rel[NP];
#pragma unroll
            for (int i = 0; i < NP; ++i) {
                const int row = stage_row<float>(i);
                rel[i] = avalid[i] ? (row >> 5) * T + (row & 31) : -1;
            }
            bx = mx8::make_bufx<float>(a.X, a.ldx, (int64_t)gt0 * T, (int64_t)B * T, rel, tid);
        }
        mx8::mainloop<float, AVEC, KFULL, !FULLT, false, BUF>(arow, avalid, wpack, K, a.k_steps / 2, wm, nt0, n_tiles_total, lds, acc, 0, 4,
                                                             &amax, &bx);
        if (dma_stage) dma_range_verdict<kLdsBytes>(amax, wpack, (int64_t)n_tiles_total * (a.k_steps / 2) * mx8::STAGE_PACK_BYTES, lds, tid & 63);
        else fused_range_verdict<kLdsBytes>(amax, wpack, (int64_t)n_tiles_total * (a.k_steps / 2) * mx8::STAGE_PACK_BYTES, lds, true);
    }
    GGCN_TRACE(5);
    if constexpr (STAMP) {
        asm volatile("" :: "v"(acc[3][RN - 1][15]));
        const unsigned long long c1 = __builtin_readcyclecounter(), w1 = __builtin_amdgcn_s_memrealtime();
        if (tid == 0 && a.stamps) {
            a.stamps[2 * (size_t)blockIdx.x] = c1 - stamp_c;
            a.stamps[2 * (size_t)blockIdx.x + 1] = w1 - stamp_w;
        }
    }
    if constexpr (((GGCN_LAB_OFF) & 128) != 0) {
        float s = 0.0f;
#pragma unroll
        for (int i = 0; i < 4; ++i)
#pragma unroll
            for (int j = 0; j < RN; ++j)
#pragma unroll
                for (int r = 0; r < 16; ++r) s += acc[i][j][r];
        if (s == 123.456f && lp.pool_a) lp.pool_a[tid] = s;
        return;
    }
    if (a.drop.thr != 0) {
        if (lp.out) epilogue<SCH, FULLT, VST, false, true, kLdsBytes, true>(a, lp, acc, g0, nt0, n_tiles_total, lds, tid);
        else epilogue<SCH, FULLT, VST, false, false, kLdsBytes, true>(a, lp, acc, g0, nt0, n_tiles_total, lds, tid);
    } else if (lp.mid) {
        if (lp.out) epilogue<SCH, FULLT, VST, true, true>(a, lp, acc, g0, nt0, n_tiles_total, lds, tid);
        else epilogue<SCH, FULLT, VST, true, false>(a, lp, acc, g0, nt0, n_tiles_total, lds, tid);
    } else {
        if (lp.out) epilogue<SCH, FULLT, VST, false, true>(a, lp, acc, g0, nt0, n_tiles_total, lds, tid);
        else epilogue<SCH, FULLT, VST, false, false>(a, lp, acc, g0, nt0, n_tiles_total, lds, tid);
    }
    GGCN_TRACE(6);
}


constexpr int kRedThreads = 1024;
__global__ __launch_bounds__(kRedThreads) void overlap_reduce_kernel(const float *__restrict__ part, int n_part, int B,
                                                                     float *__restrict__ dst)
{
    __shared__ float red[kRedThreads / 64];
    const int tid = threadIdx.x;
    float s0 = 0.0f, s1 = 0.0f, s2 = 0.0f, s3 = 0.0f;
    const int n4 = (reinterpret_cast<uintptr_t>(part) & 15u) == 0 ? n_part / 4 : 0;
    const float4 *p4 = reinterpret_cast<const float4 *>(part);
    int i = tid;
    for (; i + 3 * kRedThreads < n4; i += 4 * kRedThreads) {
        const float4 a = p4[i], b = p4[i + kRedThreads], c = p4[i + 2 * kRedThreads], d = p4[i + 3 * kRedThreads];
        s0 += (a.x + a.y) + (a.z + a.w);
        s1 += (b.x + b.y) + (b.z + b.w);
        s2 += (c.x + c.y) + (c.z + c.w);
        s3 += (d.x + d.y) + (d.z + d.w);
    }
    for (; i < n4; i += kRedThreads) {
        const float4 a = p4[i];
        s0 += (a.x + a.y) + (a.z + a.w);
    }
    for (int j = 4 * n4 + tid; j < n_part; j += kRedThreads) s1 += part[j];
    float sdot = (s0 + s1) + (s2 + s3);
#pragma unroll
    for (int d = 32; d >= 1; d >>= 1) sdot += __shfl_xor(sdot, d);
    if ((tid & 63) == 0) red[tid >> 6] = sdot;
    __syncthreads();
    if (tid == 0) {
        float t = 0.0f;
#pragma unroll
        for (int w = 0; w < kRedThreads / 64; ++w) t += red[w];
        *dst = t / (float)B;
    }
}

__global__ __launch_bounds__(256) void rowmask_kernel(const int32_t *__restrict__ rowptr,
                                                      const int32_t *__restrict__ colidx, int64_t n, int T,
                                                      uint32_t *__restrict__ rowmask)
{
    const int64_t i = (int64_t)blockIdx.x * 256 + threadIdx.x;
    if (i >= n) return;
    const int64_t base = i / T * T;
    const int W = (T + 31) >> 5;
    uint32_t m[GGCN_MASK_MAX_T / 32] = {};
    for (int e = rowptr[i]; e < rowptr[i + 1]; ++e) {
        const uint32_t j = (uint32_t)(colidx[e] - base);
#pragma unroll
        for (int w = 0; w < GGCN_MASK_MAX_T / 32; ++w)
            if ((j >> 5) == (uint32_t)w) m[w] |= 1u << (j & 31u);
    }
#pragma unroll
    for (int w = 0; w < GGCN_MASK_MAX_T / 32; ++w)
        if (w < W) rowmask[i * W + w] = m[w];
}

int launch_fused(const char *who, FusedArgs &a, int precision, hipStream_t st, bool weighted_block = false)
{
    if (precision != GGCN_PREC_BF16X3 && precision != GGCN_PREC_F16MX8 && precision != GGCN_PREC_F16MX6)
        return fail(GGCN_EUNSUPPORTED, "%s: precision %d (use bf16x3 or f16mx8)", who, precision);
#ifndef GGCN_WITH_F16MX6
    if (precision == GGCN_PREC_F16MX6)
        return fail(GGCN_EUNSUPPORTED, "%s: f16mx6 is an experiment this library was built without (make F16MX6=1); use f16mx8", who);
#endif
    if (!a.X && !a.Xb) return fail(GGCN_EINVAL, "%s: null input pointer", who);
    if (a.T > 32 ? !a.rowmask : !a.graph_ops)
        return fail(GGCN_EINVAL, "%s: graphs of %d nodes need %s", who, a.T,
                    a.T > 32 ? "the row masks" : "the per-graph operand blocks of ggcn_graph_operands");
    if (a.T <= 32 && !aligned16(a.graph_ops)) return fail(GGCN_EINVAL, "%s: graph_ops must be 16-byte aligned", who);
    if (a.T > 128 && a.graph_ops && !aligned16(a.graph_ops)) return fail(GGCN_EINVAL, "%s: the edge-list blocks must be 16-byte aligned", who);
    if (a.B <= 0 || a.T <= 0 || a.K <= 0 || a.F <= 0)
        return fail(GGCN_EINVAL, "%s: B=%d T=%d K=%d F=%d must be positive", who, a.B, a.T, a.K, a.F);
    if (a.T > GGCN_MASK_MAX_T)
        return fail(GGCN_EUNSUPPORTED, "%s: T=%d > %d; use ggcn_linear + ggcn_aggregate", who, a.T, GGCN_MASK_MAX_T);
    if (a.T > 32 && a.n_parts != 1)
        return fail(GGCN_EUNSUPPORTED, "%s: the two-layer form takes graphs of <= 32 nodes (T=%d): one ggcn_layer_fused per layer", who, a.T);
    if (a.ldx < a.K) return fail(GGCN_EINVAL, "%s: ldx < K", who);
    bool vst = true, any_out = false;
    for (int p = 0; p < a.n_parts; ++p) {
        const LayerPart &lp = a.part[p];
        if (!lp.wpack) return fail(GGCN_EINVAL, "%s: null weight image", who);
// ... 190 lines not shown
                         int B, int T, int K, int F, const float *store_gate, const float *pool_gate_a, const float *pool_gate_b,
                         float *out, int64_t ldo, float *pool_a, float *pool_b, float *overlap_partial, const float *overlap_in,
                         float *overlap_out, int precision, hipStream_t st)
{
    const char *who = "ggcn_layer_fused_weighted";
    if ((overlap_in == nullptr) != (overlap_out == nullptr)) return fail(GGCN_EINVAL, "%s: overlap_in and overlap_out go together", who);
    if (!graph_opsw || !zero_mid) return fail(GGCN_EINVAL, "%s: the weighted operand blocks and the zero row are required", who);
    if (T > 32) return fail(GGCN_EUNSUPPORTED, "%s: T=%d > 32 (use ggcn_linear + ggcn_aggregate)", who, T);
    if (precision == GGCN_PREC_F16MX6) return fail(GGCN_EUNSUPPORTED, "%s: bf16x3 or f16mx8", who);
    if (out && ldo > (int64_t)INT32_MAX) return fail(GGCN_EUNSUPPORTED, "%s: ldo too large", who);
    FusedArgs a = {};
    a.X = X; a.ldx = ldx; a.graph_ops = static_cast<const char *>(graph_opsw); a.graph_ops2 = a.graph_ops;
    a.ov_in = overlap_in; a.ov_out = overlap_out;
    a.B = B; a.T = T; a.K = K; a.F = F; a.n_parts = 1;
    a.part[0] = LayerPart{static_cast<const char *>(wpack), bias, zero_mid, nullptr, store_gate, pool_gate_a, pool_gate_b,
                          out, pool_a, pool_b, overlap_partial, (int)ldo};
    return launch_fused(who, a, precision, st);
}

int layer_fused_weighted_drop(const float *X, int64_t ldx, const void *wpack, const void *graph_opsw, const float *bias, const float *zero_mid,
                              int B, int T, int K, int F, const float *store_gate, const float *pool_gate_a, const float *pool_gate_b,
                              float *out, int64_t ldo, float *pool_a, float *pool_b, int precision, hipStream_t st, const DropSpec *drop)
{
    const char *who = "ggcn_layer_fused_weighted_drop";
    if (!graph_opsw || !zero_mid) return fail(GGCN_EINVAL, "%s: the weighted operand blocks and the zero row are required", who);
    if (!drop) return fail(GGCN_EINVAL, "%s: no keep streams", who);
    if (T > 32) return fail(GGCN_EUNSUPPORTED, "%s: T=%d > 32 (33..128 nodes: ggcn_layer_fused_weighted_wide_drop)", who, T);
    if (precision == GGCN_PREC_F16MX6) return fail(GGCN_EUNSUPPORTED, "%s: bf16x3 or f16mx8", who);
    if ((int64_t)B * T * F >= ((int64_t)1 << 32))
        return fail(GGCN_EUNSUPPORTED, "%s: gate dropout indexes elements with 32 bits (B*T*F = %lld)", who, (long long)B * T * F);
    if (out && ldo > (int64_t)INT32_MAX) return fail(GGCN_EUNSUPPORTED, "%s: ldo too large", who);
    FusedArgs a = {};
    a.X = X; a.ldx = ldx; a.graph_ops = static_cast<const char *>(graph_opsw); a.graph_ops2 = a.graph_ops;
    a.B = B; a.T = T; a.K = K; a.F = F; a.n_parts = 1;
    a.drop = *drop;
    a.part[0] = LayerPart{static_cast<const char *>(wpack), bias, zero_mid, nullptr, store_gate, pool_gate_a, pool_gate_b,
                          out, pool_a, pool_b, nullptr, (int)ldo};
    return launch_fused(who, a, precision, st);
}

int layer_fused(const float *X, int64_t ldx, const void *wpack, const uint32_t *rowmask, const void *graph_ops,
                const float *bias, int B, int T, int K, int F, const float *store_gate, const float *pool_gate_a,
                const float *pool_gate_b, float *out, int64_t ldo, float *pool_a, float *pool_b,
                float *overlap_partial, const float *overlap_in, float *overlap_out, int precision, hipStream_t st,
                const DropSpec *drop, const float *bias_pre)
{
    if ((overlap_in == nullptr) != (overlap_out == nullptr))
        return fail(GGCN_EINVAL, "ggcn_layer_fused: overlap_in and overlap_out go together");
    if (out && ldo > (int64_t)INT32_MAX) return fail(GGCN_EUNSUPPORTED, "ggcn_layer_fused: ldo too large");
    FusedArgs a = {};
    a.X = X; a.ldx = ldx; a.rowmask = rowmask; a.graph_ops = static_cast<const char *>(graph_ops);
    a.ov_in = overlap_in; a.ov_out = overlap_out;
    a.B = B; a.T = T; a.K = K; a.F = F; a.n_parts = 1;
    if (drop) a.drop = *drop;
    a.part[0] = LayerPart{static_cast<const char *>(wpack), bias, nullptr, bias_pre, store_gate, pool_gate_a, pool_gate_b,
                          out, pool_a, pool_b, overlap_partial, (int)ldo};
    if (bias_pre && T <= 32)
        return fail(GGCN_EUNSUPPORTED, "ggcn_layer_fused_prebias: graphs of <= 32 nodes fold both layers in ggcn_block_fused (its eval form); bias_pre is for 33..256 nodes");
    if (bias_pre && drop)
        return fail(GGCN_EUNSUPPORTED, "ggcn_layer_fused_prebias: an inference form (no gate dropout)");
    return launch_fused("ggcn_layer_fused", a, precision, st);
}

int layer_fused_bf16(const char *who, const void *X, int64_t ldx, const void *wpack, const uint32_t *rowmask, const void *graph_ops,
                     const float *bias, int B, int T, int K, int F,
                     const float *store_gate, const float *pool_gate_a, const float *pool_gate_b, float *out, int64_t ldo,
                     float *pool_a, float *pool_b, float *overlap_partial, const float *overlap_in, float *overlap_out,
                     hipStream_t st, const DropSpec *drop)
{
    if (!X) return fail(GGCN_EINVAL, "%s: null input pointer", who);
    if ((overlap_in == nullptr) != (overlap_out == nullptr)) return fail(GGCN_EINVAL, "%s: overlap_in and overlap_out go together", who);
    if (out && ldo > (int64_t)INT32_MAX) return fail(GGCN_EUNSUPPORTED, "%s: ldo too large", who);
    FusedArgs a = {};
    a.X = static_cast<const float *>(wpack);
    a.Xb = static_cast<const __bf16 *>(X); a.ldx = ldx; a.rowmask = rowmask; a.graph_ops = static_cast<const char *>(graph_ops);
    a.ov_in = overlap_in; a.ov_out = overlap_out;
    a.B = B; a.T = T; a.K = K; a.F = F; a.n_parts = 1;
    if (drop) a.drop = *drop;
    a.part[0] = LayerPart{static_cast<const char *>(wpack), bias, nullptr, nullptr, store_gate, pool_gate_a, pool_gate_b,
                          out, pool_a, pool_b, overlap_partial, (int)ldo};
    return launch_fused(who, a, GGCN_PREC_BF16X3, st);
}

int block_fused(const float *X, int64_t ldx, const void *wpack1, const void *wpack12, const void *graph_ops,
                const void *graph_ops2, const float *bias1, const float *bias_mid, const float *bias2, int B, int T, int K, int F,
                const float *gate1, const float *gate2, float *gcn1, int64_t ld1, float *x_out, int64_t ld2,
                float *x1, float *y1, float *pool_out, float *overlap_partial, int precision, hipStream_t st,
                unsigned long long *stamps)
{
    if (!gate2) return fail(GGCN_EINVAL, "ggcn_block_fused: gate2 is required");
    const bool layer1 = x1 || y1 || gcn1 || overlap_partial;
    if (layer1 && (!x1 || !y1 || !gate1))
        return fail(GGCN_EINVAL, "ggcn_block_fused: layer 1's outputs go together (gate1, x1 and y1; all NULL with gcn1 and overlap_partial = the eval form)");
    if (!x_out && !pool_out) return fail(GGCN_EINVAL, "ggcn_block_fused: neither x nor its pool requested");
    if ((gcn1 && ld1 > (int64_t)INT32_MAX) || (x_out && ld2 > (int64_t)INT32_MAX))
        return fail(GGCN_EUNSUPPORTED, "ggcn_block_fused: leading dimension too large");
    FusedArgs a = {};
    if (!graph_ops2 || !aligned16(graph_ops2))
        return fail(GGCN_EINVAL, "ggcn_block_fused: graph_ops2 (ggcn_graph_operands2 blocks, 16-byte aligned) is required");
    if (layer1 && !gcn1 && !stamps && precision == GGCN_PREC_F16MX8 && X && wpack1 && wpack12 && bias_mid &&
        block8_takes(X, ldx, wpack1, wpack12, B, T, K, F, gate1, gate2, bias1, bias_mid, bias2, graph_ops, graph_ops2, x_out, ld2)) {
        const char *form = getenv("GGCN_BLOCK_FORM");
        if (!(form && form[0] == '4'))
            return lab_block_fused8(X, ldx, wpack1, wpack12, graph_ops, graph_ops2, bias1, bias_mid, bias2, B, T, K, F, gate1, gate2, x_out,
                                    ld2, x1, y1, pool_out, overlap_partial, st, nullptr, kBlock8RowMajor | kBlock8Product);
    }
    a.X = X; a.ldx = ldx; a.graph_ops = static_cast<const char *>(graph_ops); a.graph_ops2 = static_cast<const char *>(graph_ops2);
    a.B = B; a.T = T; a.K = K; a.F = F; a.n_parts = layer1 ? 2 : 1;
    a.stamps = stamps;
    if (!bias_mid) return fail(GGCN_EINVAL, "ggcn_block_fused: bias_mid (W2^T.b1, zeros when gc1 has no bias) is required");
    const LayerPart second = LayerPart{static_cast<const char *>(wpack12), bias2, bias_mid, nullptr, gate2, gate2, nullptr,
                                       x_out, pool_out, nullptr, nullptr, (int)ld2};
    if (layer1) {
        a.part[0] = LayerPart{static_cast<const char *>(wpack1), bias1, nullptr, nullptr, nullptr, gate1, gate2,
                              gcn1, x1, y1, overlap_partial, (int)ld1};
        a.part[1] = second;
    } else {
        if (stamps) return fail(GGCN_EUNSUPPORTED, "ggcn_debug_block_fused_stamped: the eval form is not stamped");
        if (!a.graph_ops) a.graph_ops = a.graph_ops2;
        a.part[0] = second;
    }
    return launch_fused("ggcn_block_fused", a, precision, st);
}

int block_fused_weighted(const float *X, int64_t ldx, const void *wpack1, const void *wpack12, const void *graph_opsw,
                         const void *graph_ops2w, const float *bias1, const float *bias_mid, const float *bias2, const float *zero_mid,
                         int B, int T, int K, int F, const float *gate1, const float *gate2, float *gcn1, int64_t ld1, float *x_out,
                         int64_t ld2, float *x1, float *y1, float *pool_out, float *overlap_partial, int precision, hipStream_t st)
{
    const char *who = "ggcn_block_fused_weighted";
    if (!X) return fail(GGCN_EINVAL, "%s: null input pointer", who);
    if (T > 32) return fail(GGCN_EUNSUPPORTED, "%s: T=%d > 32 (one weighted layer launch per layer)", who, T);
    if (precision == GGCN_PREC_F16MX6) return fail(GGCN_EUNSUPPORTED, "%s: bf16x3 or f16mx8", who);
    if (!gate2) return fail(GGCN_EINVAL, "%s: gate2 is required", who);
    const bool layer1 = x1 || y1 || gcn1 || overlap_partial;
    if (layer1 && (!x1 || !y1 || !gate1))
        return fail(GGCN_EINVAL, "%s: layer 1's outputs go together (gate1, x1 and y1; all NULL with gcn1 and overlap_partial = the eval form)", who);
    if (!x_out && !pool_out) return fail(GGCN_EINVAL, "%s: neither x nor its pool requested", who);
    if ((gcn1 && ld1 > (int64_t)INT32_MAX) || (x_out && ld2 > (int64_t)INT32_MAX))
        return fail(GGCN_EUNSUPPORTED, "%s: leading dimension too large", who);
    if (!wpack12 || (layer1 && !wpack1)) return fail(GGCN_EINVAL, "%s: null weight image", who);
    if (!graph_ops2w || !aligned16(graph_ops2w))
        return fail(GGCN_EINVAL, "%s: graph_ops2w (ggcn_graph_operands2_weighted blocks, 16-byte aligned) is required", who);
    if (layer1 && (!graph_opsw || !aligned16(graph_opsw)))
        return fail(GGCN_EINVAL, "%s: layer 1 needs graph_opsw (ggcn_graph_operands_weighted blocks, 16-byte aligned)", who);
    if (!bias_mid) return fail(GGCN_EINVAL, "%s: bias_mid (W2^T.b1, zeros when gc1 has no bias) is required", who);
    if (layer1 && (!zero_mid || !aligned16(zero_mid))) return fail(GGCN_EINVAL, "%s: zero_mid ([F] zeros, 16-byte aligned) is required", who);
    FusedArgs a = {};
    a.X = X; a.ldx = ldx; a.graph_ops2 = static_cast<const char *>(graph_ops2w);
    a.graph_ops = layer1 ? static_cast<const char *>(graph_opsw) : a.graph_ops2;
    a.B = B; a.T = T; a.K = K; a.F = F; a.n_parts = layer1 ? 2 : 1;
    const LayerPart second = LayerPart{static_cast<const char *>(wpack12), bias2, bias_mid, nullptr, gate2, gate2, nullptr,
                                       x_out, pool_out, nullptr, nullptr, (int)ld2};
    if (layer1) {
        a.part[0] = LayerPart{static_cast<const char *>(wpack1), bias1, zero_mid, nullptr, nullptr, gate1, gate2,
                              gcn1, x1, y1, overlap_partial, (int)ld1};
        a.part[1] = second;
    } else {
        a.part[0] = second;
    }
    return launch_fused(who, a, precision, st, true);
}

int block_fused_bf16(const void *X, int64_t ldx, const void *wpack1, const void *wpack12, const void *graph_ops,
                     const void *graph_ops2, const float *bias1, const float *bias_mid, const float *bias2, int B, int T, int K, int F,
                     const float *gate1, const float *gate2, float *gcn1, int64_t ld1, float *x_out, int64_t ld2,
                     float *x1, float *y1, float *pool_out, float *overlap_partial, hipStream_t st)
{
    const char *who = "ggcn_block_fused_bf16";
    if (!X) return fail(GGCN_EINVAL, "%s: null input pointer", who);
    if (T > 32)
        return fail(GGCN_EUNSUPPORTED, "%s: T=%d > 32 (one ggcn_layer_fused_bf16_wide per layer up to %d nodes)", who, T, GGCN_MASK_MAX_T);
    if (!gate2) return fail(GGCN_EINVAL, "%s: gate2 is required", who);
    const bool layer1 = x1 || y1 || gcn1 || overlap_partial;
    if (layer1 && (!x1 || !y1 || !gate1))
        return fail(GGCN_EINVAL, "%s: layer 1's outputs go together (gate1, x1 and y1; all NULL with gcn1 and overlap_partial = the eval form)", who);
    if (!x_out && !pool_out) return fail(GGCN_EINVAL, "%s: neither x nor its pool requested", who);
    if ((gcn1 && ld1 > (int64_t)INT32_MAX) || (x_out && ld2 > (int64_t)INT32_MAX))
        return fail(GGCN_EUNSUPPORTED, "%s: leading dimension too large", who);
    if (!wpack12 || (layer1 && !wpack1)) return fail(GGCN_EINVAL, "%s: null weight image", who);
    if (!graph_ops2) return fail(GGCN_EINVAL, "%s: graph_ops2 (the ggcn_graph_operands2 blocks of plane 0) is required", who);
    if (!aligned16(graph_ops2)) return fail(GGCN_EINVAL, "%s: graph_ops2 must be 16-byte aligned", who);
    if (layer1 && !graph_ops) return fail(GGCN_EINVAL, "%s: layer 1 needs the per-graph operand blocks of ggcn_graph_operands", who);
    if (!bias_mid) return fail(GGCN_EINVAL, "%s: bias_mid (W2^T.b1, zeros when gc1 has no bias) is required", who);
    FusedArgs a = {};
    a.X = static_cast<const float *>(wpack12);
    a.Xb = static_cast<const __bf16 *>(X); a.ldx = ldx;
    a.graph_ops = static_cast<const char *>(graph_ops); a.graph_ops2 = static_cast<const char *>(graph_ops2);
    a.B = B; a.T = T; a.K = K; a.F = F; a.n_parts = layer1 ? 2 : 1;
// ... 26 lines not shown
```

### ed-gated-gcn_amd/dispatch.py

```python
import collections
import os

import torch

from . import _capi

BF16_PRECISIONS = ("bf16x3", "f16mx8", "f16mx6")

LAYER_PATHS = ("fused", "fused_drop", "bf16", "bf16_drop", "bf16_wide", "bf16_wide_drop", "weighted", "long", "two_launch")
DROPOUT_PATHS = ("fused_drop", "bf16_drop", "bf16_wide_drop")
OVERLAP_PATHS = LAYER_PATHS[:6]
BACKWARD_PASSES = ("mma", "one_pass", "two_pass", "two_pass_drop")
LAYER_LAUNCHES = LAYER_PATHS + ("weighted_wide", "weighted_drop", "weighted_wide_drop")
DROPOUT_LAUNCHES = DROPOUT_PATHS + ("weighted_drop", "weighted_wide_drop")
OVERLAP_LAUNCHES = OVERLAP_PATHS
BACKWARD_LAUNCHES = BACKWARD_PASSES + ("weighted", "weighted_drop")
DX_FORMS = ("bf16", "scaled", "bf16x3", "fp32")
BLOCK_PATHS = ("block", "bf16_block", "folded_eval", "bf16_folded_eval", "two_fused", "layers_eval", "layers")
BLOCK_LAUNCHES = BLOCK_PATHS + ("weighted_block",)
WEIGHTED_BLOCK_PRECISIONS = ("bf16x3", "f16mx8")


class Input(collections.namedtuple("Input", "dtype B T gpu")):
    @classmethod
# ... 130 lines not shown
    return bool(getattr(layer, "weighted_backward", False) and not csr.is_binary and csr.T <= 32 and F % 4 == 0
                and _aligned16(operands) and not _two_pass_forced() and csr.graph_ops_weighted_t() is not None)


def takes_weighted_backward(layer, csr, F, dropout, operands):
    return dropout is None and _weighted_backward_base(layer, csr, F, operands)


def takes_weighted_backward_drop(layer, csr, B, F, dropout, operands):
    return dropout is not None and B * csr.T * F < 2 ** 32 and _weighted_backward_base(layer, csr, F, operands)


def backward_launch(layer, csr, dtype, B, K, F, need_x, need_adj, dropout, operands):
    passes, dx, dw = backward_plan(layer, csr, dtype, K, F, need_x, need_adj, dropout, operands)
    if passes == "two_pass" and takes_weighted_backward(layer, csr, F, dropout, operands):
        passes = "weighted"
    elif passes == "two_pass_drop" and takes_weighted_backward_drop(layer, csr, B, F, dropout, operands):
        passes = "weighted_drop"
    return passes, dx, dw


def bf16_block_on(x, gc1):
    return bool(getattr(gc1, "bf16_block", False)) and isinstance(x, torch.Tensor) and x.is_cuda and x.dtype == torch.bfloat16


def _square(gc1, gc2):
    return gc1.out_features == gc2.in_features and gc1.out_features == gc2.out_features


def takes_block_path(x, csr, gc1, gc2):
    inp = Input.of(x)
    return (csr.T <= 32 and takes_fused(gc1, csr, inp) and takes_fused(gc2, csr, inp) and gc1.precision == gc2.precision
            and _square(gc1, gc2))


def takes_folded_eval_path(x, csr, gc1, gc2):
    inp = Input.of(x)
    return (32 < csr.T <= 256 and takes_fused(gc1, csr, inp) and takes_fused(gc2, csr, inp) and gc1.precision == gc2.precision
            and gc1.precision in ("f16mx8", "bf16x3") and _square(gc1, gc2) and gc1.in_features == gc1.out_features)


def takes_bf16_block_path(x, csr, gc1, gc2):
    return (bf16_block_on(x, gc1) and csr.T <= 32 and takes_bf16_fused(gc1, csr, Input.of(x)) and bool(gc2.fused)
            and gc1.precision in BF16_PRECISIONS and gc2.precision in BF16_PRECISIONS and _square(gc1, gc2))


def takes_bf16_folded_eval_path(x, csr, gc1, gc2):
    return (bf16_block_on(x, gc1) and 32 < csr.T <= 256 and bool(csr.is_binary) and csr.rowmask is not None
            and bool(csr.rowmask.is_cuda) and gc1.precision in BF16_PRECISIONS and takes_fused(gc2, csr, Input.of(x, torch.float32))
            and _square(gc1, gc2) and gc1.in_features == gc1.out_features)


def block_path(x, csr, gc1, gc2, want, want_gcn1, one_launch, training):
    if training:
        return "layers"
    layer1 = any(k in want for k in ("x1", "y1", "xy"))
    eval_only = not layer1 and not want_gcn1
    for name, takes, allowed in (("block", takes_block_path, True), ("bf16_block", takes_bf16_block_path, True),
                                 ("bf16_folded_eval", takes_bf16_folded_eval_path, eval_only), ("folded_eval", takes_folded_eval_path, eval_only)):
        if one_launch and allowed and takes(x, csr, gc1, gc2):
            return name
    if not layer1:
        return "layers_eval"
    inp = Input.of(x)
    if ((takes_fused(gc1, csr, inp) or takes_bf16_fused(gc1, csr, inp) or takes_bf16_wide(gc1, csr, inp))
            and takes_fused(gc2, csr, Input.of(x, torch.float32)) and gc1.out_features == gc2.out_features):
        return "two_fused"
    return "layers"


def takes_weighted_block_path(x, csr, gc1, gc2):
    if not getattr(gc1, "weighted_block", False):
        return False
    inp = Input.of(x)
    if not (inp.gpu is not None and inp.dtype == torch.float32 and not csr.is_binary and csr.T <= 32):
        return False
    if not (gc1.fused and gc2.fused and gc1.precision == gc2.precision and gc1.precision in WEIGHTED_BLOCK_PRECISIONS and _square(gc1, gc2)):
        return False
    if not (takes_weighted(gc1, csr, inp) and takes_weighted(gc2, csr, Input.of(x, torch.float32))):
        return False
    return csr.graph_ops2_weighted(0 if gc1.precision == "bf16x3" else 1) is not None


def block_launch(x, csr, gc1, gc2, want, want_gcn1, one_launch, training):
    path = block_path(x, csr, gc1, gc2, want, want_gcn1, one_launch, training)
    if path in ("layers", "layers_eval") and not training and one_launch and takes_weighted_block_path(x, csr, gc1, gc2):
        return "weighted_block"
    return path
```

### ed-gated-gcn_amd/gated_block.py

```python
import torch

from . import _capi, dispatch, range_guard
from .csr import BatchedCSR, tensor_version
from .dispatch import (takes_bf16_block_path, takes_bf16_folded_eval_path, takes_block_path, takes_folded_eval_path,
                       takes_weighted_block_path)
from .gcn import _require_gate, _rows2d

GATE_WORDING = "%(name)s must be a contiguous float32 [B,F]=[%(B)d,%(F)d] GPU tensor"


def gate_overlap(x1, y1):
    lib = _capi.load_library()
    B, F = x1.shape
    dev = x1.device
    with torch.cuda.device(dev):
        xy = torch.empty((), dtype=torch.float32, device=dev)
        ws = torch.empty(lib.ggcn_overlap_workspace_bytes(B), dtype=torch.uint8, device=dev)
        _capi.check(lib.ggcn_gate_overlap(_capi.ptr(x1), _capi.ptr(y1), B, F, _capi.ptr(xy), _capi.ptr(ws),
                                          _capi.stream_of(dev)), "ggcn_gate_overlap")
    return xy


def _block_operands(gc1, gc2, lib, st, precision=None):
    w1, w2, b1 = gc1.weight, gc2.weight, gc1.bias
# ... 23 lines not shown
        store[prec] = cached
    return gc1._packed_weight(lib, st, precision=precision), cached[1], cached[2]


def _folded_eval(x, csr, gate2, gc1, gc2, want_x):
    gc1._check(x)
    bf16 = x.dtype == torch.bfloat16
    if not bf16:
        range_guard.before(x.device)
    lib = _capi.load_library()
    (B, T, K), F, dev = x.shape, gc2.out_features, x.device
    x2d = _rows2d(x)
    _require_gate("gate2", gate2, B, F, GATE_WORDING)
    with torch.cuda.device(dev):
        st = _capi.stream_of(dev)
        prec = "bf16x3" if bf16 else gc1.precision
        _, pack12, mid = _block_operands(gc1, gc2, lib, st, precision=prec)
        z = torch.empty(B * T, K, dtype=torch.float32, device=dev)
        if bf16:
            _capi.check(lib.ggcn_aggregate_bf16(_capi.ptr(x2d), x2d.stride(0), _capi.ptr(csr.rowptr), _capi.ptr(csr.colidx),
                                                _capi.ptr(csr.vals), B, T, K, _capi.ptr(z), K, st), "ggcn_aggregate_bf16(D.A.X)")
        else:
            _capi.check(lib.ggcn_aggregate(_capi.ptr(x2d), x2d.stride(0), _capi.ptr(csr.rowptr), _capi.ptr(csr.colidx), _capi.ptr(csr.vals),
                                           None, B, T, K, None, None, None, _capi.ptr(z), K, None, None, st), "ggcn_aggregate(D.A.X)")
        xo = torch.empty(B * T, F, dtype=torch.float32, device=dev) if want_x else None
        out = torch.empty(B, F, dtype=torch.float32, device=dev)
        b2 = None if gc2.bias is None else gc2.bias.detach()
        _capi.check(lib.ggcn_layer_fused_prebias(_capi.ptr(z), K, _capi.ptr(pack12), _capi.ptr(csr.rowmask), _capi.ptr(b2), _capi.ptr(mid),
                                                 B, T, K, F, _capi.ptr(gate2), _capi.ptr(gate2), None, _capi.ptr(xo), F,
                                                 _capi.ptr(out), None, _capi.PREC[prec], st), "ggcn_layer_fused_prebias")
    if prec == "f16mx8":
        range_guard.after(x.device)
    return (None if xo is None else xo.view(B, T, F)), out


BLOCK_OUTPUTS = ("x1", "y1", "xy", "x", "out")


def gated_gcn_block(x, adj, gate1, gate2, gc1, gc2, want_gcn1=False, one_launch=True, want=None, dense_head=None):
    if dense_head is not None:
        from .heads import dense_head as _dense_head
        if torch.is_grad_enabled() and (gc1._needs_grad(x, gate1, gate2, adj=adj) or gc2._needs_grad(x, gate2, adj=adj)):
            raise RuntimeError("dense_head= is an inference feature; under autograd apply the classifier's own dense layer")
        r = _gated_gcn_block(x, adj, gate1, gate2, gc1, gc2, want_gcn1, one_launch, want, _defer_xy=True)
        part = r.pop("_xy_partials", None)
        sig = dense_head[2] if len(dense_head) > 2 else None
        if r["out"] is None:
            raise RuntimeError("dense_head= needs `out` among want=")
        if r["out"].shape[0] == 0:
            r["logits"] = r["out"].new_zeros((0, dense_head[0].shape[1]))
            return r
        if part is not None:
            r["logits"], r["xy"] = _dense_head(r["out"], dense_head[0], dense_head[1], partials=part, f_block=gc2.out_features, signal=sig)
        else:
            r["logits"] = _dense_head(r["out"], dense_head[0], dense_head[1], signal=sig)
        return r
    return _gated_gcn_block(x, adj, gate1, gate2, gc1, gc2, want_gcn1, one_launch, want)


def _one_launch_block(x, csr, gate1, gate2, gc1, gc2, want, want_gcn1, defer_xy, bf16, weighted=False):
    gc1._check(x)
    if not bf16:
        range_guard.before(x.device)
    lib = _capi.load_library()
    (B, T, K), F, dev = x.shape, gc2.out_features, x.device
    x2d = _rows2d(x)
    layer1 = want_gcn1 or any(k in want for k in ("x1", "y1", "xy"))
    if gate1 is not None or layer1:
        _require_gate("gate1", gate1, B, F, GATE_WORDING)
    _require_gate("gate2", gate2, B, F, GATE_WORDING)
    ptr, f32 = _capi.ptr, dict(dtype=torch.float32, device=dev)
    with torch.cuda.device(dev):
        st = _capi.stream_of(dev)
        kprec = "bf16x3" if bf16 else gc1.kernel_precision(x2d, csr)
        pack1, pack12, mid = _block_operands(gc1, gc2, lib, st, precision=kprec)
        gcn1 = torch.empty(B * T, F, **f32) if want_gcn1 else None
        xo = torch.empty(B * T, F, **f32) if "x" in want else None
        x1, y1 = (torch.empty(B, F, **f32), torch.empty(B, F, **f32)) if layer1 else (None, None)
        out = torch.empty(B, F, **f32)
        part = torch.empty(B, (F + 63) // 64, **f32) if "xy" in want else None
        xy = torch.empty((), **f32) if "xy" in want else None
        b1 = None if gc1.bias is None else gc1.bias.detach()
        b2 = None if gc2.bias is None else gc2.bias.detach()
        entry = "ggcn_block_fused_bf16" if bf16 else "ggcn_block_fused_weighted" if weighted else "ggcn_block_fused"
        plane = 0 if kprec == "bf16x3" else 1
        if weighted:
            ops1, ops2 = (csr.graph_ops_weighted(plane) if layer1 else None), csr.graph_ops2_weighted(plane)
            zero = (ptr(gc1._zero_row(F, dev)),)
        else:
            ops1, ops2, zero = csr.graph_ops, csr.graph_ops2(plane), ()
        _capi.check(getattr(lib, entry)(ptr(x2d), x2d.stride(0), ptr(pack1 if (layer1 or not bf16) else None), ptr(pack12),
                                        ptr(ops1), ptr(ops2), ptr(b1), ptr(mid), ptr(b2), *zero,
                                        B, T, K, F, ptr(gate1 if layer1 else None), ptr(gate2), ptr(gcn1), F, ptr(xo), F,
                                        ptr(x1), ptr(y1), ptr(out), ptr(part), *(() if bf16 else (_capi.PREC[kprec],)), st), entry)
        if part is not None and not defer_xy:
            _capi.check(lib.ggcn_overlap_reduce(ptr(part), B, F, ptr(xy), st), "ggcn_overlap_reduce")
    if kprec in ("f16mx8", "f16mx6"):
        range_guard.after(x.device)
    r = {"gcn1": None if gcn1 is None else gcn1.view(B, T, F), "x1": x1, "y1": y1, "xy": xy,
         "x": None if xo is None else xo.view(B, T, F), "out": out}
    if defer_xy and part is not None:
        r["_xy_partials"] = part
    return r


def _gated_gcn_block(x, adj, gate1, gate2, gc1, gc2, want_gcn1=False, one_launch=True, want=None, _defer_xy=False):
    want = BLOCK_OUTPUTS if want is None else tuple(want)
    bad = [k for k in want if k not in BLOCK_OUTPUTS]
    if bad:
        raise ValueError("want: unknown output(s) %s (choose from %s; gcn1 has its own flag want_gcn1)" % (bad, list(BLOCK_OUTPUTS)))
    w_x = "x" in want
    if x.shape[0] == 0:
        gc1._check(x)
        B, T, F = 0, x.shape[1], gc2.out_features
        z2 = x.new_zeros((0, F), dtype=torch.float32)
        dt = torch.float32 if dispatch.bf16_block_on(x, gc1) else x.dtype
        return {"gcn1": x.new_zeros((0, T, gc1.out_features), dtype=dt), "x1": x.new_zeros((0, gc1.out_features), dtype=dt),
                "y1": x.new_zeros((0, gc1.out_features), dtype=dt), "xy": x.new_full((), float("nan"), dtype=dt),
                "x": x.new_zeros((0, T, F), dtype=dt), "out": z2}
    csr = adj if isinstance(adj, BatchedCSR) else gc1._as_csr(adj, x)
    training = torch.is_grad_enabled() and (gc1._needs_grad(x, gate1, gate2, adj=adj) or gc2._needs_grad(x, gate2, adj=adj))
    if training and set(want) != set(BLOCK_OUTPUTS):
        raise RuntimeError("want= selects outputs of the inference block; under autograd every output is produced")
    path = dispatch.block_launch(x, csr, gc1, gc2, want, want_gcn1, one_launch, training)
    r = dict.fromkeys(("gcn1",) + BLOCK_OUTPUTS)
    if path in ("block", "bf16_block", "weighted_block"):
        r = _one_launch_block(x, csr, gate1, gate2, gc1, gc2, want, want_gcn1, _defer_xy, bf16=path == "bf16_block",
                              weighted=path == "weighted_block")
    elif path in ("folded_eval", "bf16_folded_eval"):
        r["x"], r["out"] = _folded_eval(x, csr, gate2, gc1, gc2, w_x)
    elif path == "layers_eval":
        gcn1, _, _ = gc1.forward_gated(x, csr)
        r["x"], r["out"], _ = gc2.forward_gated(gcn1, csr, store_gate=gate2, pool_gate_a=gate2, want_out=w_x, want_pool_a=True)
        r["gcn1"] = gcn1 if want_gcn1 else None
    elif path == "two_fused":
        B, F = x.shape[0], gc1.out_features
        part = torch.empty(B, (F + 63) // 64, dtype=torch.float32, device=x.device)
        r["xy"] = torch.empty((), dtype=torch.float32, device=x.device)
        r["gcn1"], r["x1"], r["y1"] = gc1.forward_gated(x, csr, store_gate=None, pool_gate_a=gate1, pool_gate_b=gate2,
                                                        want_pool_a=True, want_pool_b=True, overlap_partial=part)
        r["x"], r["out"], _ = gc2.forward_gated(r["gcn1"], csr, store_gate=gate2, pool_gate_a=gate2, want_pool_a=True,
                                                want_out=w_x, overlap_reduce=(part, r["xy"]))
    else:
        graph = adj if gc1._differentiable_adj(adj) is not None else csr
        r["gcn1"], x1, y1 = gc1.forward_gated(x, graph, store_gate=None, pool_gate_a=gate1, pool_gate_b=gate2,
                                              want_pool_a=True, want_pool_b=True)
        if torch.is_grad_enabled() and (x1.requires_grad or y1.requires_grad):
            r["xy"] = (x1 * y1).sum(1).mean()
        else:
            r["xy"] = gate_overlap(x1, y1) if "xy" in want else None
        r["x1"], r["y1"] = x1, y1
        r["x"], r["out"], _ = gc2.forward_gated(r["gcn1"], graph, store_gate=gate2, pool_gate_a=gate2,
                                                want_out=training or w_x, want_pool_a=True)
    for k in BLOCK_OUTPUTS:
        if k not in want:
            r[k] = None
    return r
```

### ed-gated-gcn_amd/range_guard.py

```python
import atexit
import sys

import torch

from . import _capi

POLL_EVERY = 16
_STATE = {}

WHAT = {
    _capi.RANGE_OVERFLOW: "a value reached fp16's range (|v| >= 65504 or infinite): results from that launch on are saturated",
    _capi.RANGE_WINDOW: "an activation left |x| <= 448, the window in which the fp8 correction terms are exact to their "
                        "format: results from that launch on have plain fp16 accuracy (2^-12 relative), outside the 1e-4 "
                        "parity with the reference's fp32 matmul (models/gcn.py:34)",
    _capi.RANGE_HIDDEN: "the one-launch layer could not rule out an fp16 overflow of its hidden values (max|x| * max_f "
                        "sum_k |w[k,f]| reached 65504): NaN outputs are possible",
}
MESSAGE = ("precision='f16mx8' on %s, in an earlier launch: %s.  Use precision='bf16x3' (full fp32 range) for this data "
           "(GraphConvolution(..., opt) with opt.ggcn_precision = 'bf16x3', or GGCN_PRECISION=bf16x3)")


def _state(dev):
    st = _STATE.get(dev.index)
    if st is None:
        st = {"flag": torch.zeros(1, dtype=torch.int32, device=dev), "host": torch.zeros(1, dtype=torch.int32).pin_memory(),
              "event": torch.cuda.Event(), "pending": False, "calls": 0}
        _STATE[dev.index] = st
    return st


def _verdict(st, dev):
    bits = int(st["host"][0])
    if bits != 0:
        st["host"].zero_()
        st["flag"].zero_()
        raise RuntimeError(MESSAGE % (dev, "; ".join(text for bit, text in WHAT.items() if bits & bit) or "flag %d" % bits))


def before(dev):
    st = _STATE.get(dev.index)
    if st is not None and st["pending"] and st["event"].query():
        st["pending"] = False
        _verdict(st, dev)


def _snapshot(st, dev):
    lib = _capi.load_library()
    with torch.cuda.device(dev):
        _capi.check(lib.ggcn_range_flag(_capi.ptr(st["flag"]), 1, _capi.stream_of(dev)), "ggcn_range_flag")


def after(dev):
    if torch.cuda.is_current_stream_capturing():
        return
    st = _state(dev)
    st["calls"] += 1
    if st["pending"] or (st["calls"] != 1 and st["calls"] % POLL_EVERY):
        return
    _snapshot(st, dev)
    with torch.cuda.device(dev):
        st["host"].copy_(st["flag"], non_blocking=True)
        st["event"].record()
    st["pending"] = True


def check(dev):
    dev = torch.device(dev)
    if dev.type != "cuda":
        raise RuntimeError("range_guard.check needs a GPU device (got %s): the flag lives in libggcn_hip.so's device memory" % (dev,))
    if dev.index is None:
        dev = torch.device("cuda", torch.cuda.current_device())
    st = _state(dev)
    _snapshot(st, dev)
    st["pending"] = False
    st["host"].copy_(st["flag"])
    _verdict(st, dev)


def reset(dev):
    dev = torch.device(dev)
    idx = torch.cuda.current_device() if dev.index is None else dev.index
    st = _STATE.get(idx)
    if st is not None:
        torch.cuda.synchronize(idx)
        st["flag"].zero_()
        st["host"].zero_()
        st["pending"] = False


def _at_exit():
    for idx in list(_STATE):
        try:
            check(torch.device("cuda", idx))
        except RuntimeError as e:
            print("ed-gated-gcn_amd: %s" % (e,), file=sys.stderr)
        except Exception:
            pass


atexit.register(_at_exit)
```

### include/ggcn.h

```cpp
#ifndef GGCN_H
#define GGCN_H

#include <stddef.h>
#include <stdint.h>

#ifdef __cplusplus
extern "C" {
#endif

#define GGCN_ABI_VERSION 14
#define GGCN_MASK_MAX_T 256

typedef void *ggcn_stream_t;

enum ggcn_status {
    GGCN_OK = 0,
    GGCN_EINVAL = 1,
    GGCN_ELAUNCH = 2,
    GGCN_EUNSUPPORTED = 3
};

enum ggcn_adj_dtype {
    GGCN_ADJ_F32 = 0,
    GGCN_ADJ_U8 = 1,
// ... 98 lines not shown
                        const float *inv,
                        const int32_t *rowptr, const int32_t *colidx, const float *vals,
                        int B, int T, int F, float *d_adj, ggcn_stream_t stream);
#define GGCN_GRAPH_OPSWT_BYTES 6144
size_t ggcn_graph_operands_weighted_t_bytes(int B);
int ggcn_graph_operands_weighted_t(const int32_t *rowptr, const int32_t *colidx, const float *vals, int B, int T,
                                   void *graph_ops_wt, int32_t *flag, ggcn_stream_t stream);
int ggcn_gate_pool_backward_weighted(const float *out, int64_t ldo, const float *store_gate, const float *gate_a,
                                     const float *gate_b, const float *d_out, int64_t ldd, const float *d_pa, const float *d_pb,
                                     const void *graph_ops_wt, const float *inv, int B, int T, int F, float *dH, int64_t ldh,
                                     float *dY, int64_t ldy, float *d_sg, float *d_ga, float *d_gb, float *d_bsum,
                                     ggcn_stream_t stream);

int ggcn_linear_h(const void *X, int64_t ldx, const void *wpack, void *Y, int64_t ldy,
                  int64_t M, int K, int F, int precision, ggcn_stream_t stream);
int ggcn_aggregate_h(const void *Hd, int64_t ldh,
                     const int32_t *rowptr, const int32_t *colidx, const float *vals,
                     const float *bias, int B, int T, int F,
                     const float *store_gate, const float *pool_gate_a, const float *pool_gate_b,
                     void *out, int64_t ldo, float *pool_a, float *pool_b,
                     ggcn_stream_t stream);

#define GGCN_LONG_MAX_T 512
int ggcn_layer_fused_h(const void *X, int64_t ldx, const void *wpack,
                       const int32_t *rowptr, const int32_t *colidx, const float *vals,
                       const float *bias, int B, int T, int K, int F,
                       const float *store_gate, const float *pool_gate_a, const float *pool_gate_b,
                       void *out, int64_t ldo, float *pool_a, float *pool_b,
                       ggcn_stream_t stream);

int ggcn_layer_fused(const float *X, int64_t ldx, const void *wpack,
                     const uint32_t *rowmask, const void *graph_ops,
                     const float *bias, int B, int T, int K, int F,
                     const float *store_gate, const float *pool_gate_a, const float *pool_gate_b,
                     float *out, int64_t ldo, float *pool_a, float *pool_b,
                     float *overlap_partial, const float *overlap_in, float *overlap_out,
                     int precision, ggcn_stream_t stream);

int ggcn_layer_fused_prebias(const float *X, int64_t ldx, const void *wpack, const uint32_t *rowmask,
                             const float *bias, const float *bias_pre, int B, int T, int K, int F,
                             const float *store_gate, const float *pool_gate_a, const float *pool_gate_b,
                             float *out, int64_t ldo, float *pool_a, float *pool_b, int precision, ggcn_stream_t stream);

int ggcn_graph_operands_weighted(const int32_t *rowptr, const int32_t *colidx, const float *vals, int B, int T, int plane,
                                 void *graph_opsw, int32_t *flag, ggcn_stream_t stream);
int ggcn_layer_fused_weighted(const float *X, int64_t ldx, const void *wpack, const void *graph_opsw, const float *bias,
                              const float *zero_mid, int B, int T, int K, int F, const float *store_gate,
                              const float *pool_gate_a, const float *pool_gate_b, float *out, int64_t ldo, float *pool_a,
                              float *pool_b, float *overlap_partial, const float *overlap_in, float *overlap_out, int precision,
                              ggcn_stream_t stream);

#define GGCN_GRAPH_OPSW_BLOCK_BYTES 4096
size_t ggcn_graph_operands_weighted_wide_bytes(int B, int T);
int ggcn_graph_operands_weighted_wide(const int32_t *rowptr, const int32_t *colidx, const float *vals, int B, int T,
                                      void *graph_opsww, int32_t *flag, ggcn_stream_t stream);
int ggcn_layer_fused_weighted_wide(const float *X, int64_t ldx, const void *wpack, const void *graph_opsww, const float *bias,
                                   int B, int T, int K, int F, const float *store_gate, const float *pool_gate_a,
                                   const float *pool_gate_b, float *out, int64_t ldo, float *pool_a, float *pool_b, int precision,
                                   ggcn_stream_t stream);

int ggcn_layer_fused_weighted_drop(const float *X, int64_t ldx, const void *wpack, const void *graph_opsw, const float *bias,
                                   const float *zero_mid, int B, int T, int K, int F, const float *store_gate,
                                   const float *pool_gate_a, const float *pool_gate_b, float *out, int64_t ldo, float *pool_a,
                                   float *pool_b, int precision, float p, uint64_t seed, int stream_store, int stream_a,
                                   int stream_b, ggcn_stream_t stream);
int ggcn_layer_fused_weighted_wide_drop(const float *X, int64_t ldx, const void *wpack, const void *graph_opsww, const float *bias,
                                        int B, int T, int K, int F, const float *store_gate, const float *pool_gate_a,
                                        const float *pool_gate_b, float *out, int64_t ldo, float *pool_a, float *pool_b,
                                        int precision, float p, uint64_t seed, int stream_store, int stream_a, int stream_b,
                                        ggcn_stream_t stream);
int ggcn_gate_pool_backward_weighted_drop(const float *out, int64_t ldo, const float *store_gate, const float *gate_a,
                                          const float *gate_b, const float *d_out, int64_t ldd, const float *d_pa,
                                          const float *d_pb, const void *graph_ops_wt, const float *inv, int B, int T, int F,
                                          float *dH, int64_t ldh, float *dY, int64_t ldy, float *d_sg, float *d_ga, float *d_gb,
                                          float *d_bsum, float p, uint64_t seed, int stream_store, int stream_a, int stream_b,
                                          ggcn_stream_t stream);

int ggcn_block_fused(const float *X, int64_t ldx, const void *wpack1, const void *wpack12,
                     const void *graph_ops, const void *graph_ops2, const float *bias1, const float *bias_mid, const float *bias2,
                     int B, int T, int K, int F, const float *gate1, const float *gate2,
                     float *gcn1, int64_t ld1, float *x_out, int64_t ld2,
                     float *x1, float *y1, float *pool_out, float *overlap_partial,
                     int precision, ggcn_stream_t stream);
int ggcn_graph_operands2_weighted(const int32_t *rowptr, const int32_t *colidx, const float *vals, int B, int T, int plane,
                                  void *graph_ops2w, int32_t *flag, ggcn_stream_t stream);
int ggcn_block_fused_weighted(const float *X, int64_t ldx, const void *wpack1, const void *wpack12,
                              const void *graph_opsw, const void *graph_ops2w, const float *bias1, const float *bias_mid,
                              const float *bias2, const float *zero_mid, int B, int T, int K, int F, const float *gate1,
                              const float *gate2, float *gcn1, int64_t ld1, float *x_out, int64_t ld2,
                              float *x1, float *y1, float *pool_out, float *overlap_partial,
                              int precision, ggcn_stream_t stream);

int ggcn_layer_fused_drop(const float *X, int64_t ldx, const void *wpack, const uint32_t *rowmask, const void *graph_ops,
                          const float *bias, int B, int T, int K, int F,
                          const float *store_gate, const float *pool_gate_a, const float *pool_gate_b,
                          float *out, int64_t ldo, float *pool_a, float *pool_b, int precision,
                          float p, uint64_t seed, int stream_store, int stream_a, int stream_b, ggcn_stream_t stream);
int ggcn_dropout_mask(int64_t rows, int F, float p, uint64_t seed, int stream_id, float *mask, ggcn_stream_t stream);

int ggcn_overlap_reduce(const float *partials, int B, int F, float *xy, ggcn_stream_t stream);

int ggcn_dense_head(const float *pooled, int64_t ldp, const float *Wt, int64_t ldw, const float *bias, int B, int H, int C,
                    float *logits, int64_t ldl, const float *overlap_partials, int F_block, float *xy, ggcn_stream_t stream);

int ggcn_dense_head_signal(const float *pooled, int64_t ldp, const float *Wt, int64_t ldw, const float *bias, int B, int H, int C,
                           float *logits, int64_t ldl, const float *overlap_partials, int F_block, float *xy, uint32_t *signal,
                           ggcn_stream_t stream);

size_t ggcn_overlap_workspace_bytes(int B);
int ggcn_gate_overlap(const float *x1, const float *y1, int B, int F, float *xy,
                      void *workspace, ggcn_stream_t stream);

int ggcn_transpose(const float *W, int rows, int cols, int64_t ldw, float *Wt, ggcn_stream_t stream);
int ggcn_gate_mlp(const float *aspect, int64_t lda, int B, int H,
                  const float *w1t_a, const float *b1_a, const float *w2t_a, const float *b2_a, float *gate_a,
                  const float *w1t_b, const float *b1_b, const float *w2t_b, const float *b2_b, float *gate_b,
                  ggcn_stream_t stream);

int ggcn_scores_head(const float *X, int64_t ldx, const float *aspect, int64_t lda,
                     const float *logits, int64_t ldl, const float *fc_weight, int64_t ldw, const float *fc_bias,
                     const float *dist, int64_t ldd, int B, int T, int H, int C,
                     float *scores, int64_t ld_scores, float *kl_part, ggcn_stream_t stream);

int ggcn_absmax(const void *X, int is_half, int64_t ld, int64_t M, int K, float *out, ggcn_stream_t stream);

enum ggcn_range_bits { GGCN_RANGE_OVERFLOW = 1, GGCN_RANGE_WINDOW = 2, GGCN_RANGE_HIDDEN = 4 };
int ggcn_range_flag(uint32_t *flag, int clear, ggcn_stream_t stream);

int ggcn_debug_poison_lds(uint32_t pattern, ggcn_stream_t stream);

int ggcn_debug_mfma_calibrate(int n_wg, int stages, uint64_t *stamps, float *sink, ggcn_stream_t stream);
int ggcn_block_fused_form(int B, int T, int K, int F);

int ggcn_lab_block_fused8(const float *X, int64_t ldx, const void *wpack1, const void *wpack12, const void *graph_ops,
                          const void *graph_ops2, const float *bias1, const float *bias_mid, const float *bias2,
                          int B, int T, int K, int F, const float *gate1, const float *gate2, float *x_out, int64_t ld2,
                          float *x1, float *y1, float *pool_out, float *overlap_partial, uint64_t *stamps, ggcn_stream_t stream);
int ggcn_debug_block_fused_stamped(const float *X, int64_t ldx, const void *wpack1, const void *wpack12,
                                   const void *graph_ops, const void *graph_ops2, const float *bias1, const float *bias_mid,
                                   const float *bias2, int B, int T, int K, int F, const float *gate1, const float *gate2,
                                   float *gcn1, int64_t ld1, float *x_out, int64_t ld2, float *x1, float *y1, float *pool_out,
                                   float *overlap_partial, int precision, uint64_t *stamps, ggcn_stream_t stream);

int ggcn_subword_pool(const float *A, int64_t sa_b, int64_t sa_r, int64_t sa_c,
                      const float *X, int64_t x_batch, int64_t ldx,
                      float *Y, int64_t y_batch, int64_t ldy,
                      int B, int R, int C, int D, ggcn_stream_t stream);
int ggcn_subword_pool_bf16(const float *A, int64_t sa_b, int64_t sa_r, int64_t sa_c,
                           const void *X, int64_t x_batch, int64_t ldx,
                           void *Y, int64_t y_batch, int64_t ldy,
                           int B, int R, int C, int D, ggcn_stream_t stream);

int ggcn_linear_bf16(const void *X, int64_t ldx, const void *wpack, float *Y, int64_t ldy,
                     int64_t M, int K, int F, ggcn_stream_t stream);
int ggcn_linear_out_bf16(const float *X, int64_t ldx, const void *wpack, void *Y, int64_t ldy,
                         int64_t M, int K, int F, ggcn_stream_t stream);
int ggcn_layer_fused_bf16(const void *X, int64_t ldx, const void *wpack, const void *graph_ops,
                          const float *bias, int B, int T, int K, int F,
                          const float *store_gate, const float *pool_gate_a, const float *pool_gate_b,
                          float *out, int64_t ldo, float *pool_a, float *pool_b,
                          float *overlap_partial, const float *overlap_in, float *overlap_out,
                          ggcn_stream_t stream);
int ggcn_layer_fused_bf16_drop(const void *X, int64_t ldx, const void *wpack, const void *graph_ops,
                               const float *bias, int B, int T, int K, int F,
                               const float *store_gate, const float *pool_gate_a, const float *pool_gate_b,
                               float *out, int64_t ldo, float *pool_a, float *pool_b,
// ... 27 lines not shown
```

Measured before the change: 843.2 million.

## Fold overlap xy reduction into block_fused launch via last-block ticket

Adds a last-arriving-workgroup tail to the fused block kernel. Each workgroup bumps a per-stream global ticket counter after writing its overlap partials with cache-bypassing stores, and the last one reduces all partials into xy. This removes the separate ggcn_overlap_reduce launch for the block path at bf16x3 and f16mx8 precision. In exchange it adds atomics, an extra barrier, a serial tail reduction in one workgroup, and host-side per-stream ticket bookkeeping behind a mutex.

```diff
diff --git a/ed-gated-gcn_amd/_capi.py b/ed-gated-gcn_amd/_capi.py
--- a/ed-gated-gcn_amd/_capi.py
+++ b/ed-gated-gcn_amd/_capi.py
@@ -39,6 +39,8 @@
                                          c_vp, c_i64, c_vp, c_vp, c_i32, c_vp]),
     "ggcn_block_fused": (c_i32, [c_vp, c_i64, c_vp, c_vp, c_vp, c_vp, c_vp, c_vp, c_vp, c_i32, c_i32, c_i32, c_i32,
                                  c_vp, c_vp, c_vp, c_i64, c_vp, c_i64, c_vp, c_vp, c_vp, c_vp, c_i32, c_vp]),
+    "ggcn_block_tail_stream_ready": (c_i32, [c_vp]),
+    "ggcn_block_tail_arm": (c_i32, [c_vp, c_vp]),
     "ggcn_graph_operands2_weighted": (c_i32, [c_vp, c_vp, c_vp, c_i32, c_i32, c_i32, c_vp, c_vp, c_vp]),
     "ggcn_block_fused_weighted": (c_i32, [c_vp, c_i64, c_vp, c_vp, c_vp, c_vp, c_vp, c_vp, c_vp, c_vp, c_i32, c_i32, c_i32, c_i32,
                                           c_vp, c_vp, c_vp, c_i64, c_vp, c_i64, c_vp, c_vp, c_vp, c_vp, c_i32, c_vp]),
@@ -122,6 +124,11 @@
 PREC = {"bf16x3": 0, "fp32": 1, "f16mx8": 2, "f16": 3, "f16mx6": 4}
 PACKED = ("bf16x3", "f16mx8", "f16", "f16mx6")
 FLAG_WEIGHTED = 1
+PREC_MASK, BLOCK_TAIL_XY = 0xff, 0x100
+
+
+def block_tail_xy_offset(B, F):
+    return (B * ((F + 63) // 64) + 3) // 4 * 4
 RANGE_OVERFLOW, RANGE_WINDOW, RANGE_HIDDEN = 1, 2, 4
 
 
diff --git a/ed-gated-gcn_amd/csrc/capi.hip b/ed-gated-gcn_amd/csrc/capi.hip
--- a/ed-gated-gcn_amd/csrc/capi.hip
+++ b/ed-gated-gcn_amd/csrc/capi.hip
@@ -205,9 +205,20 @@
                      float *x1, float *y1, float *pool_out, float *overlap_partial, int precision,
                      ggcn_stream_t stream)
 {
+    if (precision & ~(GGCN_PREC_MASK | GGCN_BLOCK_TAIL_XY)) return fail(GGCN_EINVAL, "ggcn_block_fused: unknown flag bits in precision (0x%x)", precision);
+    TailArgs tail = {};
+    if (precision & GGCN_BLOCK_TAIL_XY) {
+        if (B <= 0 || F <= 0) return fail(GGCN_EINVAL, "ggcn_block_fused: B=%d T=%d K=%d F=%d must be positive", B, T, K, F);
+        tail.xy = overlap_partial ? overlap_partial + GGCN_BLOCK_TAIL_XY_OFFSET(B, F) : nullptr;
+    }
     return block_fused(X, ldx, wpack1, wpack12, graph_ops, graph_ops2, bias1, bias_mid, bias2, B, T, K, F, gate1, gate2, gcn1, ld1,
-                       x_out, ld2, x1, y1, pool_out, overlap_partial, precision, as_stream(stream));
-}
+                       x_out, ld2, x1, y1, pool_out, overlap_partial, precision & GGCN_PREC_MASK, as_stream(stream), nullptr,
+                       (precision & GGCN_BLOCK_TAIL_XY) ? &tail : nullptr);
+}
+
+int ggcn_block_tail_stream_ready(ggcn_stream_t stream) { return block_tail_stream_ready(as_stream(stream)); }
+
+int ggcn_block_tail_arm(float *xy, ggcn_stream_t stream) { return block_tail_arm(xy, as_stream(stream)); }
 
 int ggcn_graph_operands2_weighted(const int32_t *rowptr, const int32_t *colidx, const float *vals, int B, int T, int plane,
                                   void *graph_ops2w, int32_t *flag, ggcn_stream_t stream)
@@ -553,7 +564,7 @@
 {
     if (!stamps) return fail(GGCN_EINVAL, "ggcn_debug_block_fused_stamped: null stamp buffer");
     return block_fused(X, ldx, wpack1, wpack12, graph_ops, graph_ops2, bias1, bias_mid, bias2, B, T, K, F, gate1, gate2, gcn1, ld1,
-                       x_out, ld2, x1, y1, pool_out, overlap_partial, precision, as_stream(stream),
+                       x_out, ld2, x1, y1, pool_out, overlap_partial, precision & GGCN_PREC_MASK, as_stream(stream),
                        reinterpret_cast<unsigned long long *>(stamps));
 }
 
diff --git a/ed-gated-gcn_amd/csrc/common.h b/ed-gated-gcn_amd/csrc/common.h
--- a/ed-gated-gcn_amd/csrc/common.h
+++ b/ed-gated-gcn_amd/csrc/common.h
@@ -116,11 +116,17 @@
                          int64_t ld2, float *x1, float *y1, float *pool_out, float *overlap_partial, int precision, hipStream_t st);
 int dropout_mask(int64_t rows, int F, float p, uint64_t seed, int sel, float *out, hipStream_t st);
 
+struct TailArgs {
+    unsigned *tickets;
+    float *xy;
+};
 int block_fused(const float *X, int64_t ldx, const void *wpack1, const void *wpack12, const void *graph_ops, const void *graph_ops2,
                 const float *bias1, const float *bias_mid, const float *bias2, int B, int T, int K, int F,
                 const float *gate1, const float *gate2, float *gcn1, int64_t ld1, float *x_out, int64_t ld2,
                 float *x1, float *y1, float *pool_out, float *overlap_partial, int precision, hipStream_t st,
-                unsigned long long *stamps = nullptr);
+                unsigned long long *stamps = nullptr, const TailArgs *tail = nullptr);
+int block_tail_arm(float *xy, hipStream_t st);
+int block_tail_stream_ready(hipStream_t st);
 int mfma_calibrate(int n_wg, int stages, unsigned long long *stamps, float *sink, hipStream_t st);
 int overlap_reduce(const float *partials, int B, int F, float *xy, hipStream_t st);
 
@@ -174,7 +180,7 @@
 int lab_block_fused8(const float *X, int64_t ldx, const void *wpack1, const void *wpack12, const void *graph_ops, const void *graph_ops2,
                      const float *bias1, const float *bias_mid, const float *bias2, int B, int T, int K, int F, const float *gate1,
                      const float *gate2, float *x_out, int64_t ld2, float *x1, float *y1, float *pool_out, float *overlap_partial,
-                     hipStream_t st, unsigned long long *stamps = nullptr, int flags = 0);
+                     hipStream_t st, unsigned long long *stamps = nullptr, int flags = 0, const TailArgs *tail = nullptr);
 constexpr int kBlock8RowMajor = 1, kBlock8NoDma = 2, kBlock8SameSlots = 4, kBlock8Product = 8;
 bool block8_shape(int B, int T, int K, int F);
 bool block8_takes(const float *X, int64_t ldx, const void *wpack1, const void *wpack12, int B, int T, int K, int F, const float *gate1,
diff --git a/ed-gated-gcn_amd/csrc/fused_block8.hip b/ed-gated-gcn_amd/csrc/fused_block8.hip
--- a/ed-gated-gcn_amd/csrc/fused_block8.hip
+++ b/ed-gated-gcn_amd/csrc/fused_block8.hip
@@ -6,7 +6,8 @@
 namespace {
 
 constexpr int kB8Threads = 512;
-constexpr int kB8Lds = kLdsBytes + 2 * kEpiLdsBytes;
+constexpr int kB8Tail = kLdsBytes + 2 * kEpiLdsBytes;
+constexpr int kB8Lds = kB8Tail + 16;
 
 __device__ __forceinline__ bool getenv_slot_same(const FusedArgs &a) { return (a.k_steps & 0x20000000) != 0; }
 
@@ -42,6 +43,8 @@
     }
 
     const int tid8 = threadIdx.x;
+    unsigned *tail_words = reinterpret_cast<unsigned *>(lds + kB8Tail);
+    if (a.tail.tickets && tid8 == 0) { tail_words[0] = 0u; tail_words[1] = 0u; }
     const unsigned long long t_start = a.stamps ? __builtin_amdgcn_s_memrealtime() : 0;
     const int group = __builtin_amdgcn_readfirstlane(tid8 >> 8);
     const int tid = tid8 & 255;
@@ -92,9 +95,14 @@
     mx8::range_verdict(amax, bw1, 0.0f, false);
     if (group == 0) {
         epilogue<1, FULLT, VST, false, false, kLdsBytes>(a, lp, acc, g0, nt0, n_tiles_total, lds, tid);
+        if (a.tail.tickets) tail_arrive_waves(a, tail_words, 4, tid & 63);
     } else {
         if (lp.out) epilogue<1, FULLT, VST, true, true, kLdsBytes + kEpiLdsBytes>(a, lp, acc, g0, nt0, n_tiles_total, lds, tid);
         else epilogue<1, FULLT, VST, true, false, kLdsBytes + kEpiLdsBytes>(a, lp, acc, g0, nt0, n_tiles_total, lds, tid);
+    }
+    if (a.tail.tickets) {
+        __syncthreads();
+        if (__builtin_amdgcn_readfirstlane(tail_words[1]) != 0) tail_xy(a, a.part[0].ov_partial, lds, tid8);
     }
     if (a.stamps && tid == 0) {
         unsigned long long *o = a.stamps + ((size_t)blockIdx.x * 2 + group) * 4;
@@ -138,7 +146,7 @@
 int lab_block_fused8(const float *X, int64_t ldx, const void *wpack1, const void *wpack12, const void *graph_ops, const void *graph_ops2,
                      const float *bias1, const float *bias_mid, const float *bias2, int B, int T, int K, int F, const float *gate1,
                      const float *gate2, float *x_out, int64_t ld2, float *x1, float *y1, float *pool_out, float *overlap_partial,
-                     hipStream_t st, unsigned long long *stamps, int flags)
+                     hipStream_t st, unsigned long long *stamps, int flags, const TailArgs *tail)
 {
     const char *who = (flags & kBlock8Product) ? "ggcn_block_fused" : "ggcn_lab_block_fused8";
     if (!X || !wpack1 || !wpack12 || !graph_ops || !graph_ops2 || !gate1 || !gate2 || !x1 || !y1 || !bias_mid)
@@ -157,6 +165,7 @@
     a.part[0] = LayerPart{static_cast<const char *>(wpack1), bias1, nullptr, nullptr, nullptr, gate1, gate2, nullptr, x1, y1, overlap_partial, 0};
     a.part[1] = LayerPart{static_cast<const char *>(wpack12), bias2, bias_mid, nullptr, gate2, gate2, nullptr, x_out, pool_out, nullptr, nullptr, (int)ld2};
     a.stamps = stamps;
+    if (tail) a.tail = *tail;
     a.k_steps = round_up(K, BK) / KSTEP;
     const bool al = (F % 4 == 0) && aligned16(gate1) && aligned16(gate2) && aligned16(bias1) && aligned16(bias2) && aligned16(bias_mid) &&
                     aligned16(graph_ops) && aligned16(graph_ops2) && !(flags & kBlock8NoDma);
diff --git a/ed-gated-gcn_amd/csrc/fused_common.h b/ed-gated-gcn_amd/csrc/fused_common.h
--- a/ed-gated-gcn_amd/csrc/fused_common.h
+++ b/ed-gated-gcn_amd/csrc/fused_common.h
@@ -33,6 +33,7 @@
     DropSpec drop;
     unsigned long long *stamps;
     const __bf16 *Xb;
+    TailArgs tail;
 };
 
 
@@ -336,6 +337,8 @@
 {
     return __builtin_amdgcn_make_buffer_rsrc(p, 0, 0x7fffffff, 0x00020000);
 }
+
+constexpr int kSc1 = 16;
 
 template <int SCH, bool FULLT, bool VST, bool MID, bool OUT, int BASE = kLdsBytes, bool DROP = false>
 __device__ __forceinline__ void epilogue(const FusedArgs &a, const LayerPart &lp, f32x16 (&acc)[4][RN], int g0, int nt0,
@@ -485,7 +488,8 @@
         }
         if (ov_partial && nt0 < n_tiles_total) {
             const float tot = wave_sum_to_lane0(dot);
-            if (lane == 0) ov_partial[(int64_t)g * ((F + 63) / 64) + (nt0 >> 1)] = tot;
+            if (lane == 0)
+                __builtin_amdgcn_raw_buffer_store_b32(__float_as_uint(tot), out_rsrc(ov_partial + (int64_t)g * ((F + 63) / 64)), 4 * (nt0 >> 1), 0, kSc1);
         }
         if constexpr (vst) {
             __builtin_amdgcn_fence(__ATOMIC_RELEASE, "wavefront");
@@ -510,5 +514,91 @@
 }
 
 
-}
-}
+__device__ __forceinline__ float4 tail_load4(const __amdgpu_buffer_rsrc_t &r, int byte_off)
+{
+    return __builtin_bit_cast(float4, __builtin_amdgcn_raw_buffer_load_b128(r, byte_off, 0, kSc1));
+}
+__device__ __forceinline__ float tail_load1(const __amdgpu_buffer_rsrc_t &r, int byte_off)
+{
+    return __uint_as_float(__builtin_amdgcn_raw_buffer_load_b32(r, byte_off, 0, kSc1));
+}
+
+constexpr int kTailThreads = 256, kTailDepth = 16;
+
+__device__ __forceinline__ void tail_xy(const FusedArgs &a, const float *part, char *lds, int t)
+{
+    float *red = reinterpret_cast<float *>(lds);
+    if (t < kTailThreads) {
+        const int n_part = a.B * ((a.F + 63) / 64);
+        const __amdgpu_buffer_rsrc_t pr = out_rsrc(const_cast<float *>(part));
+        float s[4] = {0.0f, 0.0f, 0.0f, 0.0f};
+        if ((reinterpret_cast<uintptr_t>(part) & 15u) == 0 && (n_part & 3) == 0) {
+            const int n4 = n_part >> 2;
+            int i = t;
+            for (; i + (kTailDepth - 1) * kTailThreads < n4; i += kTailDepth * kTailThreads) {
+                float4 p[kTailDepth];
+#pragma unroll
+                for (int q = 0; q < kTailDepth; ++q) p[q] = tail_load4(pr, (i + q * kTailThreads) * 16);
+#pragma unroll
+                for (int q = 0; q < kTailDepth; ++q) { s[0] += p[q].x; s[1] += p[q].y; s[2] += p[q].z; s[3] += p[q].w; }
+            }
+            for (; i < n4; i += kTailThreads) {
+                const float4 p = tail_load4(pr, i * 16);
+                s[0] += p.x; s[1] += p.y; s[2] += p.z; s[3] += p.w;
+            }
+        } else {
+            for (int j = 4 * t; j < n_part; j += 4 * kTailThreads)
+#pragma unroll
+                for (int e = 0; e < 4; ++e)
+                    if (j + e < n_part) s[e] += tail_load1(pr, (j + e) * 4);
+        }
+#pragma unroll
+        for (int d = 8; d >= 1; d >>= 1)
+#pragma unroll
+            for (int e = 0; e < 4; ++e) s[e] += __shfl_xor(s[e], d);
+        const float s02 = s[0] + s[2], s13 = s[1] + s[3];
+        if ((t & 15) == 0) red[t >> 4] = s02 + s13;
+    }
+    __syncthreads();
+    if (t == 0) {
+        float tot = 0.0f;
+#pragma unroll
+        for (int w = 0; w < 16; ++w) tot += red[w];
+        *a.tail.xy = tot / (float)a.B;
+    }
+}
+
+__device__ __forceinline__ bool tail_arrive_last(const FusedArgs &a)
+{
+    const unsigned old = __hip_atomic_fetch_add(a.tail.tickets, 1u, __ATOMIC_RELAXED, __HIP_MEMORY_SCOPE_AGENT);
+    if (old != (unsigned)a.g_tiles * (unsigned)a.n_wg - 1u) return false;
+    __hip_atomic_store(a.tail.tickets, 0u, __ATOMIC_RELAXED, __HIP_MEMORY_SCOPE_AGENT);
+    __builtin_amdgcn_fence(__ATOMIC_ACQUIRE, "agent");
+    asm volatile("s_waitcnt vmcnt(0)" ::: "memory");
+    return true;
+}
+
+__device__ __forceinline__ void block_tail(const FusedArgs &a, const float *part, char *lds)
+{
+    const int t = threadIdx.x;
+    asm volatile("s_waitcnt vmcnt(0)" ::: "memory");
+    __syncthreads();
+    int *flag = reinterpret_cast<int *>(lds + kLdsBytes);
+    if (t == 0) flag[0] = tail_arrive_last(a) ? 1 : 0;
+    __syncthreads();
+    if (__builtin_amdgcn_readfirstlane(flag[0]) == 0) return;
+    __syncthreads();
+    tail_xy(a, part, lds, t);
+}
+
+__device__ __forceinline__ void tail_arrive_waves(const FusedArgs &a, unsigned *words, int n_waves, int lane)
+{
+    asm volatile("s_waitcnt vmcnt(0)" ::: "memory");
+    if (lane == 0) {
+        const unsigned n = __hip_atomic_fetch_add(words, 1u, __ATOMIC_RELAXED, __HIP_MEMORY_SCOPE_WORKGROUP);
+        if (n == (unsigned)n_waves - 1u && tail_arrive_last(a)) words[1] = 1u;
+    }
+}
+
+}
+}
diff --git a/ed-gated-gcn_amd/csrc/fused_layer.hip b/ed-gated-gcn_amd/csrc/fused_layer.hip
--- a/ed-gated-gcn_amd/csrc/fused_layer.hip
+++ b/ed-gated-gcn_amd/csrc/fused_layer.hip
@@ -1,6 +1,7 @@
 #include "fused_common.h"
 
 #include <cstdlib>
+#include <mutex>
 
 namespace ggcn {
 namespace {
@@ -247,6 +248,8 @@
         else epilogue<SCH, FULLT, VST, false, false>(a, lp, acc, g0, nt0, n_tiles_total, lds, tid);
     }
     GGCN_TRACE(6);
+    if constexpr (std::is_same<XT, float>::value && !STAMP)
+        if (a.tail.tickets && !second) block_tail(a, a.part[0].ov_partial, lds);
 }
 
 
@@ -603,13 +606,85 @@
     return launch_fused(who, a, GGCN_PREC_BF16X3, st);
 }
 
+constexpr int kTailSlots = 64, kTailWords = 32, kTailDevices = 64;
+__device__ unsigned g_tail_tickets[kTailSlots * kTailWords];
+
+namespace {
+std::mutex g_tail_mu;
+unsigned *g_tail_base[kTailDevices] = {};
+hipStream_t g_tail_owner[kTailDevices][kTailSlots] = {};
+float *g_tail_armed[kTailDevices][kTailSlots] = {};
+int g_tail_used[kTailDevices] = {};
+
+bool tail_slot(hipStream_t st, bool create, int &dev, int &slot)
+{
+    if (hipGetDevice(&dev) != hipSuccess || dev < 0 || dev >= kTailDevices) { (void)hipGetLastError(); return false; }
+    for (slot = 0; slot < g_tail_used[dev]; ++slot)
+        if (g_tail_owner[dev][slot] == st) return true;
+    if (!create || g_tail_used[dev] == kTailSlots) return false;
+    if (!g_tail_base[dev]) {
+        void *p = nullptr;
+        if (hipGetSymbolAddress(&p, HIP_SYMBOL(g_tail_tickets)) != hipSuccess || !p) { (void)hipGetLastError(); return false; }
+        g_tail_base[dev] = static_cast<unsigned *>(p);
+    }
+    slot = g_tail_used[dev]++;
+    g_tail_owner[dev][slot] = st;
+    return true;
+}
+unsigned *tail_tickets_for(hipStream_t st)
+{
+    std::lock_guard<std::mutex> lock(g_tail_mu);
+    int dev, slot;
+    return tail_slot(st, true, dev, slot) ? g_tail_base[dev] + (size_t)slot * kTailWords : nullptr;
+}
+float *tail_take_armed(hipStream_t st)
+{
+    std::lock_guard<std::mutex> lock(g_tail_mu);
+    int dev, slot;
+    if (!tail_slot(st, false, dev, slot)) return nullptr;
+    float *xy = g_tail_armed[dev][slot];
+    g_tail_armed[dev][slot] = nullptr;
+    return xy;
+}
+}
+
+int block_tail_stream_ready(hipStream_t st) { return tail_tickets_for(st) != nullptr; }
+
+int block_tail_arm(float *xy, hipStream_t st)
+{
+    if (!xy) return fail(GGCN_EINVAL, "ggcn_block_tail_arm: null pointer");
+    std::lock_guard<std::mutex> lock(g_tail_mu);
+    int dev, slot;
+    if (!tail_slot(st, true, dev, slot))
+        return fail(GGCN_EUNSUPPORTED, "ggcn_block_tail_arm: no arrival word left for this stream (%d streams per device)", kTailSlots);
+    g_tail_armed[dev][slot] = xy;
+    return GGCN_OK;
+}
+
 int block_fused(const float *X, int64_t ldx, const void *wpack1, const void *wpack12, const void *graph_ops,
                 const void *graph_ops2, const float *bias1, const float *bias_mid, const float *bias2, int B, int T, int K, int F,
                 const float *gate1, const float *gate2, float *gcn1, int64_t ld1, float *x_out, int64_t ld2,
                 float *x1, float *y1, float *pool_out, float *overlap_partial, int precision, hipStream_t st,
-                unsigned long long *stamps)
-{
+                unsigned long long *stamps, const TailArgs *tail)
+{
+    TailArgs armed = {};
+    armed.xy = tail_take_armed(st);
+    if (!tail && armed.xy && !stamps) tail = &armed;
     if (!gate2) return fail(GGCN_EINVAL, "ggcn_block_fused: gate2 is required");
+    TailArgs tl = {};
+    if (tail) {
+        const char *who = "ggcn_block_fused";
+        if (stamps) return fail(GGCN_EUNSUPPORTED, "%s: the stamped form finishes nothing in the launch", who);
+        if (!x1 || !y1 || !overlap_partial || !tail->xy || gcn1)
+            return fail(GGCN_EINVAL, "%s: xy in the launch needs x1, y1, overlap_partial and xy, and takes no gcn1", who);
+        if (precision != GGCN_PREC_BF16X3 && precision != GGCN_PREC_F16MX8)
+            return fail(GGCN_EUNSUPPORTED, "%s: precision %d (xy in the launch: bf16x3 or f16mx8)", who, precision);
+        if (B > 0 && F > 0 && (int64_t)B * ((F + 63) / 64) * 4 >= ((int64_t)1 << 31))
+            return fail(GGCN_EUNSUPPORTED, "%s: xy in the launch addresses the partials with 32 bits (B=%d F=%d)", who, B, F);
+        tl = *tail;
+        tl.tickets = tail_tickets_for(st);
+        if (!tl.tickets) return fail(GGCN_EUNSUPPORTED, "%s: no arrival word left for this stream (%d streams per device)", who, kTailSlots);
+    }
     const bool layer1 = x1 || y1 || gcn1 || overlap_partial;
     if (layer1 && (!x1 || !y1 || !gate1))
         return fail(GGCN_EINVAL, "ggcn_block_fused: layer 1's outputs go together (gate1, x1 and y1; all NULL with gcn1 and overlap_partial = the eval form)");
@@ -624,8 +699,9 @@
         const char *form = getenv("GGCN_BLOCK_FORM");
         if (!(form && form[0] == '4'))
             return lab_block_fused8(X, ldx, wpack1, wpack12, graph_ops, graph_ops2, bias1, bias_mid, bias2, B, T, K, F, gate1, gate2, x_out,
-                                    ld2, x1, y1, pool_out, overlap_partial, st, nullptr, kBlock8RowMajor | kBlock8Product);
-    }
+                                    ld2, x1, y1, pool_out, overlap_partial, st, nullptr, kBlock8RowMajor | kBlock8Product, tail ? &tl : nullptr);
+    }
+    a.tail = tl;
     a.X = X; a.ldx = ldx; a.graph_ops = static_cast<const char *>(graph_ops); a.graph_ops2 = static_cast<const char *>(graph_ops2);
     a.B = B; a.T = T; a.K = K; a.F = F; a.n_parts = layer1 ? 2 : 1;
     a.stamps = stamps;
diff --git a/ed-gated-gcn_amd/dispatch.py b/ed-gated-gcn_amd/dispatch.py
--- a/ed-gated-gcn_amd/dispatch.py
+++ b/ed-gated-gcn_amd/dispatch.py
@@ -236,6 +236,24 @@
     return csr.graph_ops2_weighted(0 if gc1.precision == "bf16x3" else 1) is not None
 
 
+BLOCK_TAIL_ENV = os.environ.get("GGCN_BLOCK_TAIL", "fused")
+BLOCK_TAILS = ("launch", "xy")
+BLOCK_TAIL_PRECISIONS = ("bf16x3", "f16mx8")
+BLOCK_ENTRIES = {
+    ("block", "launch"): "ggcn_block_fused",
+    ("block", "xy"): "ggcn_block_fused",
+    ("bf16_block", "launch"): "ggcn_block_fused_bf16",
+    ("weighted_block", "launch"): "ggcn_block_fused_weighted",
+}
+
+
+def block_tail(path, kprec, wants_xy, want_gcn1, defer_xy, stream_ready):
+    if (BLOCK_TAIL_ENV == "launch" or path != "block" or kprec not in BLOCK_TAIL_PRECISIONS or not wants_xy or want_gcn1
+            or defer_xy or not stream_ready):
+        return "launch"
+    return "xy"
+
+
 def block_launch(x, csr, gc1, gc2, want, want_gcn1, one_launch, training):
     path = block_path(x, csr, gc1, gc2, want, want_gcn1, one_launch, training)
     if path in ("layers", "layers_eval") and not training and one_launch and takes_weighted_block_path(x, csr, gc1, gc2):
diff --git a/ed-gated-gcn_amd/gated_block.py b/ed-gated-gcn_amd/gated_block.py
--- a/ed-gated-gcn_amd/gated_block.py
+++ b/ed-gated-gcn_amd/gated_block.py
@@ -129,18 +129,22 @@
         xy = torch.empty((), **f32) if "xy" in want else None
         b1 = None if gc1.bias is None else gc1.bias.detach()
         b2 = None if gc2.bias is None else gc2.bias.detach()
-        entry = "ggcn_block_fused_bf16" if bf16 else "ggcn_block_fused_weighted" if weighted else "ggcn_block_fused"
+        tail = dispatch.block_tail("bf16_block" if bf16 else "weighted_block" if weighted else "block", kprec, "xy" in want, want_gcn1,
+                                   defer_xy, bool(lib.ggcn_block_tail_stream_ready(st)))
+        entry = dispatch.BLOCK_ENTRIES[("bf16_block" if bf16 else "weighted_block" if weighted else "block", tail)]
         plane = 0 if kprec == "bf16x3" else 1
         if weighted:
             ops1, ops2 = (csr.graph_ops_weighted(plane) if layer1 else None), csr.graph_ops2_weighted(plane)
             zero = (ptr(gc1._zero_row(F, dev)),)
         else:
             ops1, ops2, zero = csr.graph_ops, csr.graph_ops2(plane), ()
+        if tail == "xy":
+            _capi.check(lib.ggcn_block_tail_arm(ptr(xy), st), "ggcn_block_tail_arm")
         _capi.check(getattr(lib, entry)(ptr(x2d), x2d.stride(0), ptr(pack1 if (layer1 or not bf16) else None), ptr(pack12),
                                         ptr(ops1), ptr(ops2), ptr(b1), ptr(mid), ptr(b2), *zero,
                                         B, T, K, F, ptr(gate1 if layer1 else None), ptr(gate2), ptr(gcn1), F, ptr(xo), F,
                                         ptr(x1), ptr(y1), ptr(out), ptr(part), *(() if bf16 else (_capi.PREC[kprec],)), st), entry)
-        if part is not None and not defer_xy:
+        if part is not None and not defer_xy and tail == "launch":
             _capi.check(lib.ggcn_overlap_reduce(ptr(part), B, F, ptr(xy), st), "ggcn_overlap_reduce")
     if kprec in ("f16mx8", "f16mx6"):
         range_guard.after(x.device)
diff --git a/ed-gated-gcn_amd/range_guard.py b/ed-gated-gcn_amd/range_guard.py
--- a/ed-gated-gcn_amd/range_guard.py
+++ b/ed-gated-gcn_amd/range_guard.py
@@ -38,6 +38,8 @@
 
 
 def before(dev):
+    if torch.cuda.is_current_stream_capturing():
+        return
     st = _STATE.get(dev.index)
     if st is not None and st["pending"] and st["event"].query():
         st["pending"] = False
diff --git a/include/ggcn.h b/include/ggcn.h
--- a/include/ggcn.h
+++ b/include/ggcn.h
@@ -204,6 +204,13 @@
                      float *gcn1, int64_t ld1, float *x_out, int64_t ld2,
                      float *x1, float *y1, float *pool_out, float *overlap_partial,
                      int precision, ggcn_stream_t stream);
+
+#define GGCN_PREC_MASK 0xff
+#define GGCN_BLOCK_TAIL_XY 0x100
+#define GGCN_BLOCK_TAIL_XY_OFFSET(B, F) ((((int64_t)(B) * (((F) + 63) / 64)) + 3) / 4 * 4)
+int ggcn_block_tail_stream_ready(ggcn_stream_t stream);
+int ggcn_block_tail_arm(float *xy, ggcn_stream_t stream);
+
 int ggcn_graph_operands2_weighted(const int32_t *rowptr, const int32_t *colidx, const float *vals, int B, int T, int plane,
                                   void *graph_ops2w, int32_t *flag, ggcn_stream_t stream);
 int ggcn_block_fused_weighted(const float *X, int64_t ldx, const void *wpack1, const void *wpack12,
```

Result: no change. 843.0 million (-0.0%).
